# SandraLouise/SVJedi-graph

Measured on AMD Instinct MI355X. Metric: GAF alignments classified/sec (classify + count all-reduce + genotype, text resident in HBM), higher is better.
Workload: dtype u8/int64 (classify), f64 (likelihood)

## Files before the change

### include/svjg.h

```cpp
#ifndef SVJG_H
#define SVJG_H

#include <stdint.h>

#ifdef __cplusplus
extern "C" {
#endif

#define SVJG_ABI_VERSION 1

#define SVJG_E_NO_DEVICE   (-1)
#define SVJG_E_HIP         (-2)
#define SVJG_E_ARG         (-3)
#define SVJG_E_NOMEM       (-4)
#define SVJG_E_RCCL        (-5)
#define SVJG_E_IO          (-6)
#define SVJG_E_INPUT       (-10)
#define SVJG_E_OVERFLOW    (-12)

#define SVJG_EXC_NONE            0
#define SVJG_EXC_VALUE_ERROR     1
#define SVJG_EXC_INDEX_ERROR     2
#define SVJG_EXC_KEY_ERROR       3
#define SVJG_EXC_ZERO_DIVISION   4
#define SVJG_EXC_ASK_HOST        5
#define SVJG_EXC_TYPE_ERROR      6

typedef struct svjg_ctx svjg_ctx;

#define SVJG_LEN_UNKNOWN 0xFFFFFFFFu
#define SVJG_NODE_HAZARD 1u

typedef struct {
    uint64_t key;
    uint32_t aux;
    uint32_t row;
} svjg_node;

typedef struct {
    uint32_t right;
    uint32_t meta;
    uint32_t h0;
    uint32_t h1;
} svjg_edge;

typedef struct {
    const svjg_node *nodes;        uint64_t n_nodes;
    const svjg_edge *edges;        uint64_t n_edges;
    const uint32_t  *hits;         uint64_t n_hits;
    const char      *chrom_names;  const uint32_t *chrom_off;  const uint32_t *chrom_node_lo;  uint32_t n_chrom;
    uint32_t         n_slots;
    uint32_t         d_over;
    uint32_t         flags;
} svjg_graph;

#define SVJG_GRAPH_ALL_SLOW 1u
#define SVJG_GRAPH_DOVER_LIST 16u

typedef struct {
    uint64_t line_start;
    uint32_t slot;
    uint16_t n_ref;
    uint16_t n_alt;
} svjg_hitrec;

typedef struct {
    uint64_t n_lines;
    uint64_t n_deferred;
    uint64_t n_hitrecs;
    uint64_t non_ascii;
} svjg_stats;

int  svjg_abi_version(void);
int  svjg_device_count(void);
int  svjg_init(int device, svjg_ctx **out);
void svjg_destroy(svjg_ctx *ctx);
const char *svjg_last_error(const svjg_ctx *ctx);

int svjg_load_graph(svjg_ctx *ctx, const svjg_graph *g);
void svjg_release_host_tables(void);

int svjg_gaf_upload(svjg_ctx *ctx, const char *gaf, uint64_t n_bytes);
int svjg_gaf_upload_file(svjg_ctx *ctx, const char *path, uint64_t offset, uint64_t n_bytes);
int svjg_gaf_upload_part(svjg_ctx *ctx, const char *gaf, uint64_t n_bytes, uint64_t offset, uint64_t capacity_bytes, int last);
int svjg_classify_resident(svjg_ctx *ctx, uint64_t base_offset, int want_hits);
int svjg_classify(svjg_ctx *ctx, const char *gaf, uint64_t n_bytes, uint64_t base_offset, int want_hits);
int svjg_classify_file(svjg_ctx *ctx, const char *path, uint64_t offset, uint64_t n_bytes, int want_hits);
int svjg_reset_counts(svjg_ctx *ctx);
int svjg_get_stats(svjg_ctx *ctx, svjg_stats *out);
int svjg_input_error(svjg_ctx *ctx, int *exc_class, uint64_t *line_offset);
int svjg_get_defer_causes(svjg_ctx *ctx, uint64_t *out8);

int svjg_get_counts(svjg_ctx *ctx, uint32_t *out, uint32_t n_slots);
int svjg_set_counts(svjg_ctx *ctx, const uint32_t *in, uint32_t n_slots);
int svjg_alloc_counts(svjg_ctx *ctx, uint32_t n_slots);
int svjg_get_hits(svjg_ctx *ctx, svjg_hitrec *out, uint64_t cap, uint64_t *n);
int svjg_get_host_lines(svjg_ctx *ctx, uint64_t *out, uint64_t cap, uint64_t *n);

int svjg_comm_unique_id(char *out128);
int svjg_comm_init(svjg_ctx *ctx, const char *id128, int n_ranks, int rank);
int svjg_allreduce_counts(svjg_ctx *ctx);
int svjg_comm_init_all(svjg_ctx *const *ctxs, int n);
int svjg_comm_error(char *out, uint64_t cap);
int svjg_comm_set_stream(svjg_ctx *ctx, int second_stream);
int svjg_allreduce_counts_all(svjg_ctx *const *ctxs, int n);

int svjg_genotype(svjg_ctx *ctx, const uint8_t *sv_type, const uint32_t *slot, const uint8_t *ok,
                  uint64_t n_rows, uint32_t min_support, double err,
                  uint8_t *gt, int64_t *pl, uint32_t *raw, uint8_t *genotyped);
int svjg_genotype_boundary(svjg_ctx *ctx, uint8_t *out, uint64_t n_rows);
int svjg_genotype_view(svjg_ctx *ctx, const uint8_t *sv_type, const uint32_t *slot, const uint8_t *ok,
                       uint64_t n_rows, uint32_t min_support, double err,
                       const uint8_t **gt, const int64_t **pl, const uint32_t **raw, const uint8_t **genotyped);

int svjg_set_rows(svjg_ctx *ctx, const uint8_t *sv_type, const uint32_t *slot, const uint8_t *ok, uint64_t n_rows);
int svjg_run_resident(svjg_ctx *ctx, uint64_t base_offset, uint32_t min_support, double err,
                      const uint8_t **gt, const int32_t **pl, const uint32_t **raw, const uint8_t **flags, const uint8_t **boundary);
int svjg_run_begin(svjg_ctx *ctx, uint64_t base_offset, uint32_t min_support, double err);
int svjg_run_end(svjg_ctx *ctx, const uint8_t **gt, const int32_t **pl, const uint32_t **raw, const uint8_t **flags, const uint8_t **boundary);

int svjg_write_informative_json(const char *path, const char *gaf, uint64_t n_bytes, const svjg_hitrec *recs,
                                uint64_t n_recs, const char *const *sv_ids, uint32_t n_slots, int n_threads);

int svjg_count_informative_json(const char *path, char **keys_out, uint64_t *keys_len, uint64_t **counts_out, uint64_t *n_keys);
void svjg_host_free(void *p);

#define SVJG_E_UNSUPPORTED (-11)
typedef struct svjg_hostgraph svjg_hostgraph;
int  svjg_graph_load(const char *edges_json_path, const char *gfa_path, svjg_hostgraph **out);
const svjg_graph *svjg_graph_view(const svjg_hostgraph *g);
int  svjg_graph_info(const svjg_hostgraph *g, const char **sv_ids_blob, uint64_t *sv_ids_len, uint32_t *n_hazard);
void svjg_graph_free(svjg_hostgraph *g);

typedef struct svjg_vcf svjg_vcf;
int  svjg_vcf_load(const char *vcf_path, const char *keys_blob, uint64_t blob_len, const uint32_t *slots, uint32_t n_keys,
                   int slot_is_presence, svjg_vcf **out);
int  svjg_vcf_arrays(const svjg_vcf *v, const uint8_t **sv_type, const uint32_t **slot, const uint8_t **ok, uint64_t *n_rows);
int  svjg_vcf_write(const svjg_vcf *v, const char *out_path, const uint8_t *gt, const int64_t *pl, const uint32_t *raw,
                    const uint8_t *genotyped, uint64_t *n_genotyped);
void svjg_vcf_free(svjg_vcf *v);

int svjg_last_kernel_ms(svjg_ctx *ctx, float *classify_main_ms, float *classify_slow_ms, float *genotype_ms);
int svjg_sync(svjg_ctx *ctx);
int svjg_copy_rate(svjg_ctx *ctx, uint64_t n_bytes, double *copy_gb_per_s, double *read_gb_per_s);

#ifdef __cplusplus
}
#endif
#endif
```

### svjedi-graph_amd/csrc/svjg_capi.hip

```cpp
#include "svjg_kernels.h"
#include "svjg_host_tables.h"
#include "svjg_pass.h"
#include <rccl/rccl.h>
#include <errno.h>
#include <math.h>
#include <stdio.h>
#include <stdlib.h>
#include <string.h>
#include <fcntl.h>
#include <unistd.h>
#include <string>
#include <thread>
#include <vector>

using namespace svjg;
typedef struct svjg_ctx svjg_ctx;

static thread_local std::string g_init_error;

#include <memory>
#include <mutex>
namespace {
struct TablesCache {
    std::mutex mu;
    uint64_t key[6] = {0, 0, 0, 0, 0, 0};
    std::shared_ptr<const KernelTables> kt;
} g_tables;

uint64_t fold64(const void *p, size_t n, uint64_t h) {
    const uint8_t *b = (const uint8_t *)p;
    for (size_t i = 0; i + 8 <= n; i += 8) { uint64_t w; memcpy(&w, b + i, 8); h = (h ^ w) * 0x9E3779B97F4A7C15ull; h ^= h >> 29; }
    if (n & 7) { uint64_t w = 0; memcpy(&w, b + (n & ~(size_t)7), n & 7); h = (h ^ w ^ ((uint64_t)(n & 7) << 56)) * 0x9E3779B97F4A7C15ull; h ^= h >> 29; }
    return h;
}

uint64_t graph_digest(const svjg_graph &g, uint64_t seed) {
    uint64_t h = seed;
    h = fold64(g.nodes, (size_t)(g.n_nodes + 1) * sizeof(svjg_node), h);
    h = fold64(g.edges, (size_t)g.n_edges * sizeof(svjg_edge), h ^ g.n_edges);
    h = fold64(g.hits, (size_t)g.n_hits * sizeof(uint32_t), h ^ g.n_hits);
    h = fold64(g.chrom_off, (size_t)(g.n_chrom + 1) * sizeof(uint32_t), h ^ g.n_chrom);
    h = fold64(g.chrom_node_lo, (size_t)(g.n_chrom + 1) * sizeof(uint32_t), h);
    h = fold64(g.chrom_names, (size_t)g.chrom_off[g.n_chrom], h);
    const uint64_t tail[3] = {g.d_over, g.flags, g.n_slots};
    return fold64(tail, sizeof tail, h);
}

std::shared_ptr<const KernelTables> kernel_tables_for(const svjg_graph &g) {
    const uint64_t key[6] = {g.n_nodes, g.n_edges, g.n_hits, g.n_chrom, graph_digest(g, 1), graph_digest(g, 0xD6E8FEB86659FD93ull)};
    std::lock_guard<std::mutex> lk(g_tables.mu);
    if (!g_tables.kt || memcmp(key, g_tables.key, sizeof key) != 0) {
        g_tables.kt = std::make_shared<const KernelTables>(build_kernel_tables(g));
        memcpy(g_tables.key, key, sizeof key);
    }
    return g_tables.kt;
}
}

extern "C" void svjg_release_host_tables(void) {
    std::lock_guard<std::mutex> lk(g_tables.mu);
    g_tables.kt.reset();
    memset(g_tables.key, 0, sizeof g_tables.key);
}

constexpr int STAGE_THREADS = 4;
constexpr uint64_t STAGE_PIECE = 8ull << 20;

struct svjg_ctx {
    int device = 0;
    int n_cu = 256;
    int occ_main = 0;
    hipStream_t stream = nullptr, copy_stream = nullptr;
    hipEvent_t ev[6] = {};
    std::string err;
    bool have_graph = false, have_counts = false;
    svjg_node *d_nodes = nullptr;  svjg_edge *d_edges = nullptr;  uint32_t *d_hits = nullptr;
    uint8_t *d_cnames = nullptr;   uint32_t *d_coff = nullptr, *d_clo = nullptr, *d_chash = nullptr, *d_names = nullptr, *d_links = nullptr, *d_nok = nullptr;  uint16_t *d_disp = nullptr;  uint32_t *d_ihits = nullptr, *d_pfx = nullptr;
    GraphView gv{};
    uint32_t names_len = 0, gflags = 0, n_slots = 0;
    unsigned long long *d_counts = nullptr, *d_snap = nullptr;
    uint8_t *d_gaf = nullptr;  uint64_t gaf_cap = 0, gaf_bytes = 0;  bool have_gaf = false;
    char *h_stage[STAGE_THREADS * 2] = {};
    hipStream_t stage_stream[STAGE_THREADS] = {};
    hipEvent_t stage_ev[STAGE_THREADS * 2] = {};
    uint64_t *d_deferred = nullptr;  uint64_t deferred_cap = 0;
    svjg_hitrec *d_recs = nullptr;   uint64_t rec_cap = 0;
    uint64_t *d_host = nullptr;      uint64_t host_cap = 0;
    DevStatus *d_st = nullptr;
    unsigned long long *d_dbg = nullptr;
    uint32_t *d_long = nullptr;
    DevStatus *h_stp = nullptr;
    DevStatus &hs() { return *h_stp; }
    uint64_t total_deferred = 0;
    dd *d_logfact = nullptr;  uint32_t logfact_n = 0;  dd *d_bsum = nullptr;
    unsigned int *d_maxn = nullptr;
    void *d_rows = nullptr;  uint64_t rows_cap = 0;
    void *h_rows = nullptr;  uint64_t h_rows_cap = 0;
    uint64_t geno_rows = 0;
    struct RunSlot {
        void *d = nullptr;  uint64_t d_cap = 0;  void *h = nullptr;  uint64_t h_cap = 0;  void *h_dev = nullptr;
        unsigned long long *counts = nullptr;  uint64_t counts_cap = 0;
        hipEvent_t ev[6] = {};  hipEvent_t computed = nullptr, copied = nullptr;
        uint64_t base_offset = 0;  uint32_t min_support = 0;  double err = 0;  bool had_text = false, slow_end_own = false;
    } run[2];
    int run_head = 0, run_tail = 0, run_inflight = 0;
    int counts_in_slot = -1;
    void *d_run_in = nullptr;  uint64_t d_run_in_cap = 0;  uint64_t run_rows = 0;  bool have_rows = false;
    float ms_main = 0, ms_slow = 0, ms_geno = 0;
    ncclComm_t comm = nullptr;
    bool allreduce_second = false;
    uint64_t part_total = 0, part_need = 0, part_next = 0;
};

#define HIPCHK(ctx, call)                                                                         \
    do {                                                                                          \
        hipError_t e_ = (call);                                                                   \
        if (e_ != hipSuccess) {                                                                   \
            (ctx)->err = std::string(#call) + ": " + hipGetErrorString(e_);                       \
            return SVJG_E_HIP;                                                                    \
        }                                                                                         \
    } while (0)

extern "C" int svjg_abi_version(void) { return SVJG_ABI_VERSION; }

extern "C" int svjg_device_count(void) {
    int n = 0;
    if (hipGetDeviceCount(&n) != hipSuccess) return 0;
    return n;
}

extern "C" const char *svjg_last_error(const svjg_ctx *ctx) { return ctx ? ctx->err.c_str() : g_init_error.c_str(); }

extern "C" int svjg_init(int device, svjg_ctx **out) {
    if (!out) return SVJG_E_ARG;
    *out = nullptr;
    int n = 0;
    hipError_t e = hipGetDeviceCount(&n);
    if (e != hipSuccess || n <= 0) {
        g_init_error = "no HIP device visible (libsvjg_hip has no CPU fallback)";
        return SVJG_E_NO_DEVICE;
    }
    if (device < 0 || device >= n) { g_init_error = "device index out of range"; return SVJG_E_ARG; }
    svjg_ctx *c = new svjg_ctx();
    c->device = device;
    if (hipSetDevice(device) != hipSuccess || hipStreamCreate(&c->stream) != hipSuccess) {
        g_init_error = "hipSetDevice / hipStreamCreate failed";
        delete c;
        return SVJG_E_HIP;
    }
    hipDeviceProp_t prop;
    if (hipGetDeviceProperties(&prop, device) == hipSuccess) c->n_cu = prop.multiProcessorCount;
    for (auto &ev : c->ev) hipEventCreate(&ev);
    if (hipMalloc(&c->d_dbg, 32 * 8) != hipSuccess || hipMalloc(&c->d_st, sizeof(DevStatus)) != hipSuccess || hipMalloc(&c->d_maxn, sizeof(unsigned int)) != hipSuccess ||
        hipHostMalloc((void **)&c->h_stp, 2 * sizeof(DevStatus), hipHostMallocDefault) != hipSuccess) {
        g_init_error = "hipMalloc failed";
        delete c;
        return SVJG_E_NOMEM;
    }
    memset(c->h_stp, 0, 2 * sizeof(DevStatus));
    c->h_stp[1].err = ~0ull;
    hipFuncSetAttribute((const void *)k_classify_main, hipFuncAttributeMaxDynamicSharedMemorySize, 160 * 1024);
    *out = c;
    return 0;
}

static void free_graph(svjg_ctx *c) {
    hipFree(c->d_nodes); hipFree(c->d_edges); hipFree(c->d_hits); hipFree(c->d_cnames); hipFree(c->d_coff);
    hipFree(c->d_clo); hipFree(c->d_chash); hipFree(c->d_counts); hipFree(c->d_snap); hipFree(c->d_names); hipFree(c->d_links); hipFree(c->d_disp); hipFree(c->d_ihits); hipFree(c->d_nok); hipFree(c->d_pfx);
    c->d_pfx = nullptr; c->d_nok = nullptr; c->d_names = nullptr; c->d_links = nullptr; c->d_disp = nullptr; c->d_ihits = nullptr;
    c->d_nodes = nullptr; c->d_edges = nullptr; c->d_hits = nullptr; c->d_cnames = nullptr; c->d_coff = nullptr;
    c->d_clo = nullptr; c->d_chash = nullptr; c->d_counts = nullptr; c->d_snap = nullptr;
    c->have_graph = false; c->have_counts = false;
}

extern "C" void svjg_destroy(svjg_ctx *c) {
    if (!c) return;
    hipSetDevice(c->device);
    if (c->stream) hipStreamSynchronize(c->stream);
    if (c->copy_stream) hipStreamSynchronize(c->copy_stream);
    if (c->comm) ncclCommDestroy(c->comm);
    free_graph(c);
    hipFree(c->d_long);
    hipFree(c->d_gaf); hipFree(c->d_deferred); hipFree(c->d_recs); hipFree(c->d_host); hipFree(c->d_st); hipFree(c->d_logfact);
    hipFree(c->d_bsum); hipFree(c->d_maxn); hipFree(c->d_rows); hipFree(c->d_run_in);
    for (auto &r : c->run) {
        hipFree(r.d); hipFree(r.counts);
        if (r.h) hipHostFree(r.h);
        for (auto &e : r.ev) if (e) hipEventDestroy(e);
        if (r.computed) hipEventDestroy(r.computed);
        if (r.copied) hipEventDestroy(r.copied);
    }
    if (c->h_rows) hipHostFree(c->h_rows);
    if (c->h_stp) hipHostFree(c->h_stp);
    for (auto &b : c->h_stage) if (b) hipHostFree(b);
    for (auto &ev : c->stage_ev) if (ev) hipEventDestroy(ev);
    for (auto &st : c->stage_stream) if (st) hipStreamDestroy(st);
    for (auto &ev : c->ev) if (ev) hipEventDestroy(ev);
    if (c->copy_stream) hipStreamDestroy(c->copy_stream);
    if (c->stream) hipStreamDestroy(c->stream);
    delete c;
}

template <class T>
static int upload(svjg_ctx *c, T **dst, const T *src, uint64_t n, uint64_t extra = 0) {
    HIPCHK(c, hipMalloc((void **)dst, (n + extra + 1) * sizeof(T)));
    if (n) HIPCHK(c, hipMemcpyAsync(*dst, src, n * sizeof(T), hipMemcpyHostToDevice, c->stream));
    return 0;
}

#ifndef SVJG_SMALL_CHUNK
#define SVJG_SMALL_CHUNK 65536
#endif
#ifndef SVJG_FIRST_SHARE
#define SVJG_FIRST_SHARE 0.85
#endif
constexpr uint64_t SMALL_CHUNK = SVJG_SMALL_CHUNK;
constexpr double FIRST_CHUNK_SHARE = SVJG_FIRST_SHARE;

static int reset_status(svjg_ctx *c, bool all) {
    if (all) {
        c->hs() = c->h_stp[1]; c->total_deferred = 0;
        HIPCHK(c, hipMemcpyAsync(c->d_st, &c->h_stp[1], sizeof(DevStatus), hipMemcpyHostToDevice, c->stream));
        return 0;
    }
    c->hs().n_deferred = 0; c->hs().overflow = 0; c->hs().next_chunk = 0;
    HIPCHK(c, hipMemcpyAsync(c->d_st, &c->hs(), sizeof(DevStatus), hipMemcpyHostToDevice, c->stream));
    return 0;
}

extern "C" int svjg_load_graph(svjg_ctx *c, const svjg_graph *g) {
    if (!c || !g || !g->nodes || !g->chrom_off || !g->chrom_node_lo) return SVJG_E_ARG;
    if (g->n_nodes >= 0x7FFFFFFFull || g->n_edges >= 0x7FFFFFFFull || g->n_chrom >= 65535) { c->err = "graph too large"; return SVJG_E_ARG; }
    if (g->d_over >= 0x80000000u) { c->err = "d_over too large"; return SVJG_E_ARG; }
    HIPCHK(c, hipSetDevice(c->device));
    free_graph(c);
    int rc;
    struct Undo { svjg_ctx *c; bool armed = true; ~Undo() { if (armed) { hipStreamSynchronize(c->stream); free_graph(c); } } } undo{c};
    if ((rc = upload(c, &c->d_nodes, g->nodes, g->n_nodes + 1))) return rc;
    if ((rc = upload(c, &c->d_edges, g->edges, g->n_edges))) return rc;
    if ((rc = upload(c, &c->d_hits, g->hits, g->n_hits))) return rc;
    c->names_len = g->chrom_off[g->n_chrom];
    if ((rc = upload(c, &c->d_cnames, (const uint8_t *)g->chrom_names, c->names_len, 8))) return rc;
    if ((rc = upload(c, &c->d_coff, g->chrom_off, g->n_chrom + 1))) return rc;
    if ((rc = upload(c, &c->d_clo, g->chrom_node_lo, g->n_chrom + 1))) return rc;
    std::vector<uint32_t> hash = build_chrom_hash(*g);
    if ((rc = upload(c, &c->d_chash, hash.data(), hash.size()))) return rc;
    const std::shared_ptr<const KernelTables> ktp = kernel_tables_for(*g);
    const KernelTables &kt = *ktp;
    if ((rc = upload(c, &c->d_names, kt.names.data(), kt.names.size()))) return rc;
    if ((rc = upload(c, &c->d_links, kt.links.data(), kt.links.size()))) return rc;
    if ((rc = upload(c, &c->d_disp, kt.disp.data(), kt.disp.size()))) return rc;
    if ((rc = upload(c, &c->d_ihits, kt.ihits.data(), kt.ihits.size()))) return rc;
    if ((rc = upload(c, &c->d_nok, kt.node_of_kid.data(), kt.node_of_kid.size()))) return rc;
    if (!kt.name_pfx.empty() && (rc = upload(c, &c->d_pfx, kt.name_pfx.data(), kt.name_pfx.size()))) return rc;
    HIPCHK(c, hipStreamSynchronize(c->stream));
    c->gv.nodes = c->d_nodes; c->gv.n_nodes = (uint32_t)g->n_nodes; c->gv.edges = c->d_edges; c->gv.hits = c->d_hits;
    c->gv.chrom_names = c->d_cnames; c->gv.chrom_off = c->d_coff; c->gv.chrom_lo = c->d_clo; c->gv.chrom_hash = c->d_chash;
    c->gv.n_chrom = g->n_chrom; c->gv.hash_mask = (uint32_t)hash.size() - 1; c->gv.d_over = g->d_over;
    c->gv.dover_list = (g->flags & SVJG_GRAPH_DOVER_LIST) ? 1u : 0u;
    c->gv.name_pfx = c->d_pfx;
    c->gv.node_of_kid = c->d_nok; c->gv.name_tab = c->d_names; c->gv.name_ihits = c->d_ihits; c->gv.name_disp = c->d_disp; c->gv.name_slots = kt.name_slots; c->gv.name_buckets = kt.name_buckets;
    c->gv.name_complete = (kt.names_left_out == 0 && kt.names_skipped == 0) ? 1u : 0u;
    c->gv.link_tab = c->d_links; c->gv.link_mask = kt.link_mask; c->gv.link_seed = kt.link_seed;
    c->gflags = g->flags;
    if (g->flags & SVJG_GRAPH_DOVER_LIST) c->gflags |= SVJG_GRAPH_ALL_SLOW;
    if (kt.links_left_out) c->gflags |= SVJG_GRAPH_ALL_SLOW;
    c->n_slots = g->n_slots;
    HIPCHK(c, hipMalloc((void **)&c->d_counts, ((uint64_t)g->n_slots + GUARD_WORDS) * 8));
    HIPCHK(c, hipMalloc((void **)&c->d_snap, ((uint64_t)g->n_slots + GUARD_WORDS) * 8));
    c->have_graph = true; c->have_counts = true;
    undo.armed = false;
    return svjg_reset_counts(c);
}

extern "C" int svjg_alloc_counts(svjg_ctx *c, uint32_t n_slots) {
    if (!c) return SVJG_E_ARG;
    HIPCHK(c, hipSetDevice(c->device));
    free_graph(c);
    c->n_slots = n_slots;
    HIPCHK(c, hipMalloc((void **)&c->d_counts, ((uint64_t)n_slots + GUARD_WORDS) * 8));
    HIPCHK(c, hipMalloc((void **)&c->d_snap, ((uint64_t)n_slots + GUARD_WORDS) * 8));
    c->have_counts = true;
    return svjg_reset_counts(c);
}

extern "C" int svjg_reset_counts(svjg_ctx *c) {
    if (!c || !c->have_counts) return SVJG_E_ARG;
    c->counts_in_slot = -1;
    HIPCHK(c, hipSetDevice(c->device));
    HIPCHK(c, hipMemsetAsync(c->d_counts, 0, ((uint64_t)c->n_slots + GUARD_WORDS) * 8, c->stream));
    return reset_status(c, true);
}

static int gaf_reserve(svjg_ctx *c, uint64_t n, uint64_t *need_out) {
    const uint64_t need = ((n + 15) & ~15ull) + TEXT + 64;
    if (need > c->gaf_cap) {
        HIPCHK(c, hipStreamSynchronize(c->stream));
        hipFree(c->d_gaf); c->d_gaf = nullptr; c->gaf_cap = 0;
        HIPCHK(c, hipMalloc((void **)&c->d_gaf, need));
        c->gaf_cap = need;
    }
    *need_out = need;
    return 0;
}

static int staged_upload(svjg_ctx *c, int fd, uint64_t offset, uint64_t n, uint64_t dst_off = 0) {
    for (int i = 0; i < STAGE_THREADS * 2; ++i) {
        if (!c->h_stage[i]) HIPCHK(c, hipHostMalloc((void **)&c->h_stage[i], STAGE_PIECE, hipHostMallocDefault));
        if (!c->stage_ev[i]) HIPCHK(c, hipEventCreateWithFlags(&c->stage_ev[i], hipEventDisableTiming));
    }
    for (int t = 0; t < STAGE_THREADS; ++t)
        if (!c->stage_stream[t]) HIPCHK(c, hipStreamCreateWithFlags(&c->stage_stream[t], hipStreamNonBlocking));
    const uint64_t n_pieces = (n + STAGE_PIECE - 1) / STAGE_PIECE;
    std::string errs[STAGE_THREADS];
    int rcs[STAGE_THREADS] = {};
    auto feeder = [&](int t) {
        auto fail = [&](int rc, const std::string &m) { rcs[t] = rc; errs[t] = m; };
        if (hipSetDevice(c->device) != hipSuccess) return fail(SVJG_E_HIP, "hipSetDevice in an ingest thread");
        bool used[2] = {false, false};
        uint64_t k = 0;
        for (uint64_t p = (uint64_t)t; p < n_pieces && !rcs[t]; p += STAGE_THREADS, ++k) {
            const int b = t * 2 + (int)(k & 1);
            const uint64_t a = p * STAGE_PIECE, len = n - a < STAGE_PIECE ? n - a : STAGE_PIECE;
            if (used[k & 1] && hipEventSynchronize(c->stage_ev[b]) != hipSuccess) return fail(SVJG_E_HIP, "hipEventSynchronize (ingest)");
            for (uint64_t got = 0; got < len;) {
                const ssize_t r = pread(fd, c->h_stage[b] + got, len - got, (off_t)(offset + a + got));
                if (r <= 0) return fail(SVJG_E_IO, r == 0 ? "the GAF file is shorter than announced" : std::string("pread: ") + strerror(errno));
                got += (uint64_t)r;
            }
            if (hipMemcpyAsync(c->d_gaf + dst_off + a, c->h_stage[b], len, hipMemcpyHostToDevice, c->stage_stream[t]) != hipSuccess ||
                hipEventRecord(c->stage_ev[b], c->stage_stream[t]) != hipSuccess) return fail(SVJG_E_HIP, "hipMemcpyAsync (ingest)");
            used[k & 1] = true;
        }
        if (hipStreamSynchronize(c->stage_stream[t]) != hipSuccess) fail(SVJG_E_HIP, "hipStreamSynchronize (ingest)");
    };
    std::vector<std::thread> th;
    for (int t = 1; t < STAGE_THREADS; ++t) th.emplace_back(feeder, t);
    feeder(0);
    for (auto &x : th) x.join();
    for (int t = 0; t < STAGE_THREADS; ++t)
        if (rcs[t]) { c->err = errs[t]; return rcs[t]; }
    return 0;
}

static uint32_t lane_blocks_per_cu(svjg_ctx *c) {
    static int per_cu = 0;
    if (!per_cu) {
        int n = 0;
        if (hipOccupancyMaxActiveBlocksPerMultiprocessor(&n, k_classify_slow, (int)SLOW_TPB, 0) != hipSuccess || n < 1) n = 4;
        per_cu = n;
    }
    (void)c;
    return (uint32_t)per_cu;
}

static int gaf_finish(svjg_ctx *c, uint64_t n, uint64_t need) {
    HIPCHK(c, hipMemsetAsync(c->d_gaf + n, 0, need - n, c->stream));
    HIPCHK(c, hipStreamSynchronize(c->stream));
    c->gaf_bytes = n;
    c->have_gaf = true;
    return 0;
}

extern "C" int svjg_gaf_upload(svjg_ctx *c, const char *gaf, uint64_t n) {
    if (!c || (n && !gaf)) return SVJG_E_ARG;
    if (c->run_inflight) { c->err = "svjg_gaf_upload with a pass in flight (svjg_run_end first: a repeat of that pass would read the new text)"; return SVJG_E_ARG; }
    HIPCHK(c, hipSetDevice(c->device));
    uint64_t need;
    int rc = gaf_reserve(c, n, &need);
    if (rc) return rc;
    c->have_gaf = false;
    if (n) HIPCHK(c, hipMemcpyAsync(c->d_gaf, gaf, n, hipMemcpyHostToDevice, c->stream));
    return gaf_finish(c, n, need);
}

extern "C" int svjg_gaf_upload_part(svjg_ctx *c, const char *gaf, uint64_t n, uint64_t offset, uint64_t capacity, int last) {
    if (!c || (n && !gaf) || n > capacity || offset > capacity - n) return SVJG_E_ARG;
    if (c->run_inflight) { c->err = "svjg_gaf_upload_part with a pass in flight (svjg_run_end first)"; return SVJG_E_ARG; }
    HIPCHK(c, hipSetDevice(c->device));
    if (offset == 0) {
        int rc = gaf_reserve(c, capacity, &c->part_need);
        if (rc) return rc;
        c->have_gaf = false; c->part_total = capacity; c->part_next = 0;
    }
    if (capacity != c->part_total || offset != c->part_next || c->have_gaf) { c->err = "svjg_gaf_upload_part: pieces go in ascending order, the first at offset 0"; return SVJG_E_ARG; }
    if (n) HIPCHK(c, hipMemcpyAsync(c->d_gaf + offset, gaf, n, hipMemcpyHostToDevice, c->stream));
    HIPCHK(c, hipStreamSynchronize(c->stream));
    c->part_next = offset + n;
    if (last) return gaf_finish(c, c->part_next, c->part_need);
    return 0;
}

extern "C" int svjg_gaf_upload_file(svjg_ctx *c, const char *path, uint64_t offset, uint64_t n) {
    if (!c || !path) return SVJG_E_ARG;
    if (c->run_inflight) { c->err = "svjg_gaf_upload_file with a pass in flight (svjg_run_end first)"; return SVJG_E_ARG; }
    HIPCHK(c, hipSetDevice(c->device));
    uint64_t need;
    int rc = gaf_reserve(c, n, &need);
    if (rc) return rc;
    c->have_gaf = false;
    if (n) {
        const int fd = open(path, O_RDONLY | O_CLOEXEC);
        if (fd < 0) { c->err = std::string("open ") + path + ": " + strerror(errno); return SVJG_E_IO; }
        rc = staged_upload(c, fd, offset, n);
        close(fd);
        if (rc) return rc;
    }
    return gaf_finish(c, n, need);
}

static int ensure(svjg_ctx *c, void **p, uint64_t *cap, uint64_t want, size_t elem, bool keep) {
    if (want <= *cap) return 0;
    const uint64_t asked = want;
    if (keep && *cap && want < *cap + *cap / 2) want = *cap + *cap / 2;
    void *q = nullptr;
    if (want != asked && hipMalloc(&q, want * elem) != hipSuccess) { (void)hipGetLastError(); q = nullptr; want = asked; }
    if (!q) HIPCHK(c, hipMalloc(&q, want * elem));
    if (keep && *p && *cap) HIPCHK(c, hipMemcpyAsync(q, *p, *cap * elem, hipMemcpyDeviceToDevice, c->stream));
    HIPCHK(c, hipStreamSynchronize(c->stream));
    hipFree(*p);
    *p = q; *cap = want;
    return 0;
}

static int fetch_slot_counts(svjg_ctx *c) {
    if (c->counts_in_slot < 0) return 0;
    const int k = c->counts_in_slot;
    c->counts_in_slot = -1;
    HIPCHK(c, hipSetDevice(c->device));
    if (c->run[k].copied) HIPCHK(c, hipStreamWaitEvent(c->stream, c->run[k].copied, 0));
    HIPCHK(c, hipMemcpyAsync(c->d_counts, c->run[k].counts, ((uint64_t)c->n_slots + GUARD_WORDS) * 8, hipMemcpyDeviceToDevice, c->stream));
    return 0;
}

static uint64_t deferred_want(const svjg_ctx *c, uint64_t n) { return (c->gflags & SVJG_GRAPH_ALL_SLOW) ? n / 24 + 64 : (n / 4096 + 65536); }

static void main_launch_setup(svjg_ctx *c, uint64_t begin, uint64_t end, uint64_t base_offset, int want_hits, ClassifyArgs &a, uint32_t &grid, size_t &lds) {
    const uint64_t n = end - begin;
    const bool all_slow = (c->gflags & SVJG_GRAPH_ALL_SLOW) != 0;
    a.gaf = c->d_gaf; a.begin = begin; a.n_bytes = end; a.base_offset = base_offset; a.g = c->gv;
    a.all_slow = all_slow; a.want_hits = want_hits != 0;
#ifdef SVJG_ABLATE
    { const char *dg = getenv("SVJG_DIAG"); a.diag = dg ? (uint32_t)atoi(dg) : 0u; }
#endif
    a.counts = c->d_counts; a.deferred = c->d_deferred; a.deferred_cap = c->deferred_cap;
    a.recs = c->d_recs; a.rec_cap = c->rec_cap; a.host_lines = c->d_host; a.host_cap = c->host_cap; a.st = c->d_st; a.dbg = c->d_dbg;
    lds = LDS_MAIN;
    if (c->occ_main < 1) {
        int occ = 0;
        if (hipOccupancyMaxActiveBlocksPerMultiprocessor(&occ, k_classify_main, (int)WG, lds) != hipSuccess || occ < 1) occ = 1;
        const int by_lds = (int)((160u * 1024u) / ((lds + LDS_GRANULE - 1) / LDS_GRANULE * LDS_GRANULE));
        if (by_lds >= 1 && occ > by_lds) occ = by_lds;
        c->occ_main = occ;
        hipFree(c->d_long); c->d_long = nullptr;
#ifdef SVJG_ABLATE
        { const char *oc = getenv("SVJG_OCC"); fprintf(stderr, "[svjg diag] occupancy API: %d workgroups of %u threads per CU (LDS %zu)\n", occ, WG, lds); if (oc && atoi(oc) > 0) c->occ_main = atoi(oc); }
#endif
    }
    const uint64_t full = (uint64_t)c->n_cu * (uint64_t)c->occ_main;
    if (!c->d_long && hipMalloc((void **)&c->d_long, full * LONG_WORDS * sizeof(uint32_t)) != hipSuccess) c->d_long = nullptr;
    a.long_pre = c->d_long;
    const uint64_t share = (n + full - 1) / full;
    uint64_t region = (share + 15) & ~15ull;
    a.small = 0;
    if (share >= 8 * SMALL_CHUNK) { region = ((uint64_t)(share * FIRST_CHUNK_SHARE) + 15) & ~15ull; a.small = SMALL_CHUNK; }
    if (region < TEXT) region = TEXT;
    a.region = region;
    const uint64_t want_grid = (n + region - 1) / region;
    grid = (uint32_t)(want_grid < full ? want_grid : full);
}

static int classify_range(svjg_ctx *c, uint64_t begin, uint64_t end, uint64_t base_offset, int want_hits) {
    HIPCHK(c, hipSetDevice(c->device));
    { const int rc0 = fetch_slot_counts(c); if (rc0) return rc0; }
    if (end <= begin) return 0;
    const uint64_t n = end - begin;
    uint64_t def_want = deferred_want(c, n);
    uint64_t rec_want = want_hits ? c->hs().n_recs + n / 40 + 65536 : 0;
    uint64_t host_want = c->hs().n_host + 4096;
    int rc;
    for (int attempt = 0; attempt < 3; ++attempt) {
        if ((rc = ensure(c, (void **)&c->d_deferred, &c->deferred_cap, def_want, sizeof(uint64_t), false))) return rc;
        if ((rc = ensure(c, (void **)&c->d_host, &c->host_cap, host_want, sizeof(uint64_t), true))) return rc;
        if (want_hits && (rc = ensure(c, (void **)&c->d_recs, &c->rec_cap, rec_want, sizeof(svjg_hitrec), true))) return rc;
        HIPCHK(c, hipMemcpyAsync(c->d_snap, c->d_counts, ((uint64_t)c->n_slots + GUARD_WORDS) * 8, hipMemcpyDeviceToDevice, c->stream));
        DevStatus before = c->hs();
        if ((rc = reset_status(c, false))) return rc;
        ClassifyArgs a{};
        uint32_t grid = 0;
        size_t lds = 0;
        main_launch_setup(c, begin, end, base_offset, want_hits, a, grid, lds);
        if (!a.long_pre) { c->err = "no memory for the workers' scratch words"; return SVJG_E_NOMEM; }
#ifdef SVJG_TIMING
        if (a.diag & 16u) HIPCHK(c, hipMemsetAsync(c->d_dbg, 0, 32 * 8, c->stream));
#endif
        HIPCHK(c, hipEventRecord(c->ev[0], c->stream));
        hipLaunchKernelGGL(k_classify_main, dim3(grid), dim3(WG), lds, c->stream, a);
        HIPCHK(c, hipGetLastError());
        HIPCHK(c, hipEventRecord(c->ev[1], c->stream));
        HIPCHK(c, hipMemcpyAsync(&c->hs(), c->d_st, sizeof(DevStatus), hipMemcpyDeviceToHost, c->stream));
        HIPCHK(c, hipStreamSynchronize(c->stream));
        const uint64_t n_def = c->hs().n_deferred;
#ifdef SVJG_TIMING
        if (a.diag & 16u) {
            unsigned long long d[16];
            HIPCHK(c, hipMemcpy(d, c->d_dbg, sizeof d, hipMemcpyDeviceToHost));
// ... 283 lines not shown
    std::lock_guard<std::mutex> lk(g_comm_err_mu);
    const size_t n = g_comm_err.size() < cap - 1 ? g_comm_err.size() : (size_t)cap - 1;
    memcpy(out, g_comm_err.data(), n); out[n] = 0;
    return 0;
}

extern "C" int svjg_comm_init_all(svjg_ctx *const *ctxs, int n) {
    if (!ctxs || n < 1 || n > 64) return SVJG_E_ARG;
    for (int i = 0; i < n; ++i) if (!ctxs[i]) return SVJG_E_ARG;
    if (n == 1) return 0;
    int devs[64];
    ncclComm_t comms[64];
    for (int i = 0; i < n; ++i) {
        devs[i] = ctxs[i]->device;
        for (int j = 0; j < i; ++j) if (devs[j] == devs[i]) { comm_err_set("svjg_comm_init_all: one context per device"); return SVJG_E_ARG; }
    }
    ncclResult_t r = ncclCommInitAll(comms, n, devs);
    if (r != ncclSuccess) { comm_err_set(std::string("ncclCommInitAll: ") + ncclGetErrorString(r)); return SVJG_E_RCCL; }
    for (int i = 0; i < n; ++i) {
        if (ctxs[i]->comm) ncclCommDestroy(ctxs[i]->comm);
        ctxs[i]->comm = comms[i];
    }
    return 0;
}

extern "C" int svjg_allreduce_counts_all(svjg_ctx *const *ctxs, int n) {
    if (!ctxs || n < 1 || n > 64) return SVJG_E_ARG;
    for (int i = 0; i < n; ++i) {
        if (!ctxs[i] || !ctxs[i]->have_counts || ctxs[i]->n_slots != ctxs[0]->n_slots) return SVJG_E_ARG;
        if (n > 1 && !ctxs[i]->comm) { ctxs[0]->err = "svjg_comm_init_all has not been called"; return SVJG_E_ARG; }
    }
    int rc;
    for (int i = 0; i < n; ++i) if ((rc = fetch_slot_counts(ctxs[i])) || (rc = launch_guard(ctxs[i]))) { if (i) ctxs[0]->err = ctxs[i]->err; return rc; }
    if (n > 1) {
        ncclResult_t r = ncclGroupStart();
        for (int i = 0; i < n && r == ncclSuccess; ++i) {
            svjg_ctx *c = ctxs[i];
            if (hipSetDevice(c->device) != hipSuccess) { ctxs[0]->err = "hipSetDevice"; ncclGroupEnd(); return SVJG_E_HIP; }
            r = ncclAllReduce(c->d_counts, c->d_counts, (size_t)c->n_slots + GUARD_WORDS, ncclUint64, ncclSum, c->comm, c->stream);
        }
        const ncclResult_t r2 = ncclGroupEnd();
        if (r == ncclSuccess) r = r2;
        if (r != ncclSuccess) { ctxs[0]->err = std::string("ncclAllReduce (group): ") + ncclGetErrorString(r); return SVJG_E_RCCL; }
    }
    for (int i = 0; i < n; ++i) if ((rc = check_guard(ctxs[i]))) { if (i) ctxs[0]->err = ctxs[i]->err; return rc; }
    return 0;
}


static int build_logfact(svjg_ctx *c, uint32_t upto) {
    if (upto > LOGFACT_CAP) upto = LOGFACT_CAP;
    const uint32_t want = (upto + LF_BLOCK - 1) / LF_BLOCK * LF_BLOCK;
    hipFree(c->d_logfact); hipFree(c->d_bsum); c->d_logfact = nullptr; c->d_bsum = nullptr; c->logfact_n = 0;
    HIPCHK(c, hipMalloc((void **)&c->d_logfact, (uint64_t)want * sizeof(dd)));
    HIPCHK(c, hipMalloc((void **)&c->d_bsum, (uint64_t)(want / LF_BLOCK) * sizeof(dd)));
    hipLaunchKernelGGL(k_logfact_local, dim3(want / LF_BLOCK), dim3(LF_BLOCK), 0, c->stream, c->d_logfact, c->d_bsum, want);
    hipLaunchKernelGGL(k_logfact_bsum, dim3(1), dim3(64), 0, c->stream, c->d_bsum, want / LF_BLOCK);
    hipLaunchKernelGGL(k_logfact_add, dim3(want / LF_BLOCK), dim3(LF_BLOCK), 0, c->stream, c->d_logfact, c->d_bsum, want);
    HIPCHK(c, hipGetLastError());
    c->logfact_n = want;
    return 0;
}

static int genotype_rows(svjg_ctx *c, const uint8_t *sv_type, const uint32_t *slot, const uint8_t *ok, uint64_t n_rows,
                         uint32_t min_support, double err) {
    HIPCHK(c, hipSetDevice(c->device));
    { const int rc0 = fetch_slot_counts(c); if (rc0) return rc0; }
    const uint64_t out_bytes = n_rows * 35, maxn_off = (out_bytes + 7) & ~7ull, in_off = maxn_off + 8, in_bytes = n_rows * 6;
    const uint64_t total = in_off + in_bytes + 64;
    int rc = ensure(c, &c->d_rows, &c->rows_cap, total, 1, false);
    if (rc) return rc;
    if (total > c->h_rows_cap) {
        if (c->h_rows) hipHostFree(c->h_rows);
        c->h_rows = nullptr; c->h_rows_cap = 0;
        HIPCHK(c, hipHostMalloc(&c->h_rows, total, hipHostMallocDefault));
        c->h_rows_cap = total;
    }
    uint8_t *base = (uint8_t *)c->d_rows, *hb = (uint8_t *)c->h_rows;
    int64_t *d_pl = (int64_t *)base;
    uint32_t *d_raw = (uint32_t *)(base + n_rows * 24);
    uint8_t *d_gt = base + n_rows * 32, *d_done = base + n_rows * 33;
    unsigned int *d_maxn = (unsigned int *)(base + maxn_off);
    uint32_t *d_slot = (uint32_t *)(base + in_off);
    uint8_t *d_type = base + in_off + n_rows * 4, *d_ok = base + in_off + n_rows * 5;
    memcpy(hb + in_off, slot, n_rows * 4); memcpy(hb + in_off + n_rows * 4, sv_type, n_rows); memcpy(hb + in_off + n_rows * 5, ok, n_rows);
    HIPCHK(c, hipMemcpyAsync(base + in_off, hb + in_off, in_bytes, hipMemcpyHostToDevice, c->stream));
    GenoArgs a{};
    a.counts = c->d_counts; a.sv_type = d_type; a.slot = d_slot; a.ok = d_ok; a.n_rows = n_rows; a.min_support = min_support;
    a.l_ok = log10(1.0 - err); a.l_err = log10(err); a.l_half = log10(1.0 / 2.0);
    a.gt = d_gt; a.pl = d_pl; a.raw = d_raw; a.genotyped = d_done; a.boundary = base + n_rows * 34; a.max_n = d_maxn; a.n_slots = c->n_slots;
    c->geno_rows = n_rows;
    const uint32_t grid = (uint32_t)((n_rows + TPB - 1) / TPB);
    HIPCHK(c, hipEventRecord(c->ev[4], c->stream));
    uint32_t grow_to = 65536;
    for (int attempt = 0; attempt < 2; ++attempt) {
        if (c->logfact_n == 0 && (rc = build_logfact(c, grow_to))) return rc;
        a.logfact = c->d_logfact; a.logfact_n = c->logfact_n;
        HIPCHK(c, hipMemsetAsync(d_maxn, 0, 8, c->stream));
        hipLaunchKernelGGL(k_genotype, dim3(grid), dim3(TPB), 0, c->stream, a);
        HIPCHK(c, hipGetLastError());
        if (attempt == 0) HIPCHK(c, hipEventRecord(c->ev[5], c->stream));
        HIPCHK(c, hipMemcpyAsync(hb, base, maxn_off + 8, hipMemcpyDeviceToHost, c->stream));
        HIPCHK(c, hipStreamSynchronize(c->stream));
        if (*(const unsigned int *)(hb + maxn_off + 4)) { c->err = "slot out of range"; return SVJG_E_ARG; }
        const unsigned int max_n = *(const unsigned int *)(hb + maxn_off);
        if (max_n == 0) break;
        if (attempt == 1) { c->err = "log10(i!) table could not be sized"; return SVJG_E_HIP; }
        grow_to = max_n < LOGFACT_CAP - 1024 ? max_n + 1 + 1024 : LOGFACT_CAP;
        c->logfact_n = 0;
    }
    HIPCHK(c, hipEventElapsedTime(&c->ms_geno, c->ev[4], c->ev[5]));
    return 0;
}

extern "C" int svjg_genotype(svjg_ctx *c, const uint8_t *sv_type, const uint32_t *slot, const uint8_t *ok, uint64_t n_rows,
                             uint32_t min_support, double err, uint8_t *gt, int64_t *pl, uint32_t *raw, uint8_t *genotyped) {
    if (!c || !c->have_counts) return SVJG_E_ARG;
    if (n_rows == 0) return 0;
    if (!sv_type || !slot || !ok || !gt || !pl || !raw || !genotyped) return SVJG_E_ARG;
    const int rc = genotype_rows(c, sv_type, slot, ok, n_rows, min_support, err);
    if (rc) return rc;
    const uint8_t *hb = (const uint8_t *)c->h_rows;
    memcpy(pl, hb, n_rows * 24); memcpy(raw, hb + n_rows * 24, n_rows * 8);
    memcpy(gt, hb + n_rows * 32, n_rows); memcpy(genotyped, hb + n_rows * 33, n_rows);
    return 0;
}

extern "C" int svjg_genotype_view(svjg_ctx *c, const uint8_t *sv_type, const uint32_t *slot, const uint8_t *ok, uint64_t n_rows,
                                  uint32_t min_support, double err, const uint8_t **gt, const int64_t **pl, const uint32_t **raw,
                                  const uint8_t **genotyped) {
    if (!c || !c->have_counts || !gt || !pl || !raw || !genotyped) return SVJG_E_ARG;
    *gt = nullptr; *pl = nullptr; *raw = nullptr; *genotyped = nullptr;
    if (n_rows == 0) return 0;
    if (!sv_type || !slot || !ok) return SVJG_E_ARG;
    const int rc = genotype_rows(c, sv_type, slot, ok, n_rows, min_support, err);
    if (rc) return rc;
    const uint8_t *hb = (const uint8_t *)c->h_rows;
    *pl = (const int64_t *)hb; *raw = (const uint32_t *)(hb + n_rows * 24);
    *gt = hb + n_rows * 32; *genotyped = hb + n_rows * 33;
    return 0;
}

struct RunLayout { uint64_t pl32, raw, gt, flags, boundary, h_tail, out_bytes;  uint64_t maxn, status, guard, tail_bytes, pl64, total; };
static RunLayout run_layout(uint64_t n) {
    RunLayout L; uint64_t o = 0;
    L.pl32 = o; o += n * 12; L.raw = o; o += n * 8; L.gt = o; o += n; L.flags = o; o += n; L.boundary = o; o += n; o = (o + 63) & ~63ull; L.h_tail = o;
    uint64_t d = 0;
    L.maxn = d; d += 8; L.status = d; d += (sizeof(DevStatus) + 7) & ~7ull; L.guard = d; d += GUARD_WORDS * 8; L.tail_bytes = d;
    L.out_bytes = L.h_tail + L.tail_bytes;
    d = (d + 63) & ~63ull; L.pl64 = d; d += n * 24; L.total = d + 64;
    return L;
}

extern "C" int svjg_set_rows(svjg_ctx *c, const uint8_t *sv_type, const uint32_t *slot, const uint8_t *ok, uint64_t n_rows) {
    if (!c || (n_rows && (!sv_type || !slot || !ok))) return SVJG_E_ARG;
    if (c->run_inflight) { c->err = "svjg_set_rows with a pass in flight"; return SVJG_E_ARG; }
    if (!c->have_counts) { c->err = "svjg_set_rows needs the count vector (svjg_load_graph / svjg_alloc_counts first)"; return SVJG_E_ARG; }
    { const int rc0 = fetch_slot_counts(c); if (rc0) return rc0; }
    HIPCHK(c, hipSetDevice(c->device));
    const RunLayout L = run_layout(n_rows);
    int rc;
    if ((rc = ensure(c, &c->d_run_in, &c->d_run_in_cap, n_rows * 6 + 64, 1, false))) return rc;
    for (int k = 0; k < 2; ++k) {
        svjg_ctx::RunSlot &r = c->run[k];
        if ((rc = ensure(c, &r.d, &r.d_cap, L.total, 1, false))) return rc;
        if (L.out_bytes > r.h_cap) {
            if (r.h) hipHostFree(r.h);
            r.h = nullptr; r.h_cap = 0;
            HIPCHK(c, hipHostMalloc(&r.h, L.out_bytes, hipHostMallocMapped));
            r.h_cap = L.out_bytes;
            HIPCHK(c, hipHostGetDevicePointer(&r.h_dev, r.h, 0));
        }
        if ((rc = ensure(c, (void **)&r.counts, &r.counts_cap, (uint64_t)c->n_slots + GUARD_WORDS, sizeof(unsigned long long), false))) return rc;
        for (auto &e : r.ev) if (!e) HIPCHK(c, hipEventCreate(&e));
        if (!r.computed) HIPCHK(c, hipEventCreate(&r.computed));
        if (!r.copied) HIPCHK(c, hipEventCreateWithFlags(&r.copied, hipEventDisableTiming));
    }
    if (!c->copy_stream) {
        int least = 0, greatest = 0;
        if (hipDeviceGetStreamPriorityRange(&least, &greatest) != hipSuccess) least = 0;
        HIPCHK(c, hipStreamCreateWithPriority(&c->copy_stream, hipStreamNonBlocking, least));
    }
    uint8_t *in = (uint8_t *)c->d_run_in;
    if (n_rows) {
        HIPCHK(c, hipMemcpyAsync(in, slot, n_rows * 4, hipMemcpyHostToDevice, c->stream));
        HIPCHK(c, hipMemcpyAsync(in + n_rows * 4, sv_type, n_rows, hipMemcpyHostToDevice, c->stream));
        HIPCHK(c, hipMemcpyAsync(in + n_rows * 5, ok, n_rows, hipMemcpyHostToDevice, c->stream));
    }
    HIPCHK(c, hipStreamSynchronize(c->stream));
    c->run_rows = n_rows; c->have_rows = true;
    return 0;
}

static GenoArgs run_geno_args(svjg_ctx *c, const svjg_ctx::RunSlot &r, const RunLayout &L, uint32_t min_support, double err, const unsigned long long *counts) {
    uint8_t *base = (uint8_t *)r.d, *hostb = (uint8_t *)r.h_dev;
    const uint8_t *in = (const uint8_t *)c->d_run_in;
    GenoArgs a{};
    a.counts = counts; a.slot = (const uint32_t *)in; a.sv_type = in + c->run_rows * 4; a.ok = in + c->run_rows * 5; a.n_rows = c->run_rows;
    a.min_support = min_support;
    a.l_ok = log10(1.0 - err); a.l_err = log10(err); a.l_half = log10(1.0 / 2.0);
    a.gt = hostb + L.gt; a.pl = (int64_t *)(base + L.pl64); a.raw = (uint32_t *)(hostb + L.raw); a.genotyped = hostb + L.flags;
    a.pl32 = (int32_t *)(hostb + L.pl32); a.boundary = hostb + L.boundary; a.max_n = (unsigned int *)(base + L.maxn); a.n_slots = c->n_slots;
    a.logfact = c->d_logfact; a.logfact_n = c->logfact_n;
    return a;
}

extern "C" int svjg_run_begin(svjg_ctx *c, uint64_t base_offset, uint32_t min_support, double err) {
    if (!c) return SVJG_E_ARG;
    if (!c->have_graph || !c->have_gaf) { c->err = "svjg_run_begin needs a graph and an uploaded GAF"; return SVJG_E_ARG; }
    if (!c->have_rows) { c->err = "svjg_set_rows has not been called"; return SVJG_E_ARG; }
    if (c->run_inflight >= 2) { c->err = "two passes are in flight: svjg_run_end first"; return SVJG_E_ARG; }
    HIPCHK(c, hipSetDevice(c->device));
    const uint64_t n = c->gaf_bytes, n_rows = c->run_rows;
    const RunLayout L = run_layout(n_rows);
    svjg_ctx::RunSlot &r = c->run[c->run_head];
    int rc;
    if ((rc = ensure(c, (void **)&c->d_deferred, &c->deferred_cap, deferred_want(c, n), sizeof(uint64_t), false))) return rc;
    if ((rc = ensure(c, (void **)&c->d_host, &c->host_cap, 4096, sizeof(uint64_t), false))) return rc;
    if (c->logfact_n == 0 && (rc = build_logfact(c, 65536))) return rc;
    r.base_offset = base_offset; r.min_support = min_support; r.err = err;
    uint8_t *base = (uint8_t *)r.d;
    DevStatus *d_st = (DevStatus *)(base + L.status);
    if (r.counts_cap < (uint64_t)c->n_slots + GUARD_WORDS) { c->err = "svjg_set_rows must follow svjg_load_graph"; return SVJG_E_ARG; }
    GenoArgs ga = run_geno_args(c, r, L, min_support, err, r.counts);
    {
        const uint64_t words = (uint64_t)c->n_slots + GUARD_WORDS;
        uint32_t rg = (uint32_t)((words + TPB - 1) / TPB);
        if (rg > 1024) rg = 1024;
        hipLaunchKernelGGL(k_step_reset, dim3(rg), dim3(TPB), 0, c->stream, r.counts, words, d_st, ga.max_n);
    }
    const uint64_t max_blocks = (uint64_t)c->n_cu * 4, wave_limit = 16 * max_blocks;
    if (n) {
        ClassifyArgs a{};
        uint32_t grid = 0;
        size_t lds = 0;
        main_launch_setup(c, 0, n, base_offset, 0, a, grid, lds);
        if (!a.long_pre) { c->err = "no memory for the workers' scratch words"; return SVJG_E_NOMEM; }
        a.st = d_st; a.counts = r.counts;
        HIPCHK(c, hipEventRecord(r.ev[0], c->stream));
        hipLaunchKernelGGL(k_classify_main, dim3(grid), dim3(WG), lds, c->stream, a);
        HIPCHK(c, hipEventRecord(r.ev[1], c->stream));
        hipLaunchKernelGGL(k_classify_slow_wave, dim3((uint32_t)c->n_cu), dim3(SLOW_TPB), 0, c->stream, a, SLOW_ASK_DEVICE, 0ull, wave_limit);
        const uint64_t lane_blocks = (uint64_t)c->n_cu * lane_blocks_per_cu(c);
        hipLaunchKernelGGL(k_classify_slow, dim3((uint32_t)lane_blocks), dim3(SLOW_TPB), 0, c->stream, a, SLOW_ASK_DEVICE, wave_limit, ~0ull - 1);
        HIPCHK(c, hipGetLastError());
    }
    static const bool env_second = [] { const char *e = getenv("SVJG_ALLREDUCE_STREAM"); return e && !strcmp(e, "second"); }();
    const bool allreduce_second = env_second || c->allreduce_second;
    auto reduce_on = [&](hipStream_t st) -> int {
        int rc2 = launch_guard(c, r.counts, st, d_st);
        if (rc2) return rc2;
        ncclResult_t nr = ncclAllReduce(r.counts, r.counts, (size_t)c->n_slots + GUARD_WORDS, ncclUint64, ncclSum, c->comm, st);
        if (nr != ncclSuccess) { c->err = std::string("ncclAllReduce: ") + ncclGetErrorString(nr); return SVJG_E_RCCL; }
        HIPCHK(c, hipMemcpyAsync(base + L.guard, r.counts + c->n_slots, GUARD_WORDS * 8, hipMemcpyDeviceToDevice, st));
        return 0;
    };
    r.slow_end_own = false;
    if (c->comm && !allreduce_second) {
        if (r.had_text) { HIPCHK(c, hipEventRecord(r.ev[2], c->stream)); r.slow_end_own = true; }
        if ((rc = reduce_on(c->stream))) return rc;
    }
    HIPCHK(c, hipEventRecord(r.computed, c->stream));
    HIPCHK(c, hipStreamWaitEvent(c->copy_stream, r.computed, 0));
    if (c->comm && allreduce_second && (rc = reduce_on(c->copy_stream))) return rc;
    if (n_rows) {
        HIPCHK(c, hipEventRecord(r.ev[4], c->copy_stream));
        uint32_t gb = 64, gg = (uint32_t)c->n_cu;
        { const char *e = getenv("SVJG_GENO_BLOCK"); if (e && atoi(e) > 0) gb = (uint32_t)atoi(e); }
        { const char *e = getenv("SVJG_GENO_GRID"); if (e && atoi(e) > 0) gg = (uint32_t)atoi(e); }
        if (gb > TPB) gb = TPB;
        if ((uint64_t)gg * gb > n_rows + gb) gg = (uint32_t)((n_rows + gb - 1) / gb);
        hipLaunchKernelGGL(k_genotype, dim3(gg), dim3(gb), 0, c->copy_stream, ga);
        HIPCHK(c, hipGetLastError());
        HIPCHK(c, hipEventRecord(r.ev[5], c->copy_stream));
    }
    HIPCHK(c, hipMemcpyAsync((uint8_t *)r.h + L.h_tail, r.d, L.tail_bytes, hipMemcpyDeviceToHost, c->copy_stream));
    HIPCHK(c, hipEventRecord(r.copied, c->copy_stream));
    c->counts_in_slot = c->run_head;
    r.had_text = n != 0;
    c->run_head ^= 1; ++c->run_inflight;
    return 0;
}

extern "C" int svjg_run_end(svjg_ctx *c, const uint8_t **gt, const int32_t **pl, const uint32_t **raw, const uint8_t **flags, const uint8_t **boundary) {
    if (!c || !gt || !pl || !raw || !flags || !boundary) return SVJG_E_ARG;
    *gt = nullptr; *pl = nullptr; *raw = nullptr; *flags = nullptr; *boundary = nullptr;
    if (!c->run_inflight) { c->err = "no pass in flight"; return SVJG_E_ARG; }
    HIPCHK(c, hipSetDevice(c->device));
    svjg_ctx::RunSlot &r = c->run[c->run_tail];
    c->run_tail ^= 1; --c->run_inflight;
    const uint64_t n = c->gaf_bytes, n_rows = c->run_rows;
    const RunLayout L = run_layout(n_rows);
    uint8_t *hb = (uint8_t *)r.h;
    int rc;
    HIPCHK(c, hipEventSynchronize(r.copied));
    const uint8_t *tail = hb + L.h_tail;
    c->hs() = *(const DevStatus *)(tail + L.status);
    c->ms_slow = 0;
    if (r.had_text) {
        HIPCHK(c, hipEventElapsedTime(&c->ms_main, r.ev[0], r.ev[1]));
        if (c->hs().n_deferred) HIPCHK(c, hipEventElapsedTime(&c->ms_slow, r.ev[1], r.slow_end_own ? r.ev[2] : r.computed));
    }
    if (n_rows) HIPCHK(c, hipEventElapsedTime(&c->ms_geno, r.ev[4], r.ev[5]));
    bool again = false;
    const unsigned long long *redo_counts = r.counts;
    const unsigned long long *gd = (const unsigned long long *)(tail + L.guard);
    if (pass_repeats(c->comm != nullptr, c->hs().overflow, gd[GUARD_REPEAT])) {
        if ((rc = svjg_reset_counts(c))) return rc;
        rc = classify_range(c, 0, n, r.base_offset, 0);
        if (rc && rc != SVJG_E_INPUT) return rc;
        if (c->comm) { const std::string keep = c->err; const int rc2 = svjg_allreduce_counts(c); if (rc2 && !rc) return rc2; if (rc) c->err = keep; }
        if (rc) return rc;
        again = true; redo_counts = c->d_counts;
    } else {
        c->total_deferred = c->hs().n_deferred;
        if (c->hs().err != ~0ull) return SVJG_E_INPUT;
        if (c->comm && pass_counts_overflowed(gd[GUARD_MAX_REF], gd[GUARD_MAX_ALT])) { c->err = "more than 2^32 informative alignments for one SV"; return SVJG_E_OVERFLOW; }
    }
    if (c->hs().n_host) { c->err = "the text holds lines only the host can decide (non-ASCII digits in a decimal column: svjg_get_host_lines); classify it with svjg_classify"; return SVJG_E_ARG; }
    if (n_rows) {
        for (int attempt = 0;; ++attempt) {
            if (!again) {
                if (*(const unsigned int *)(tail + L.maxn + 4)) { c->err = "slot out of range"; return SVJG_E_ARG; }
                const unsigned int max_n = *(const unsigned int *)(tail + L.maxn);
                if (max_n == 0) break;
                if (attempt == 2) { c->err = "log10(i!) table could not be sized"; return SVJG_E_HIP; }
                HIPCHK(c, hipStreamSynchronize(c->stream));
                HIPCHK(c, hipStreamSynchronize(c->copy_stream));
                if ((rc = build_logfact(c, max_n < LOGFACT_CAP - 1024 ? max_n + 1 + 1024 : LOGFACT_CAP))) return rc;
            }
            again = false;
            GenoArgs ga = run_geno_args(c, r, L, r.min_support, r.err, redo_counts);
            HIPCHK(c, hipMemsetAsync(ga.max_n, 0, 8, c->stream));
            hipLaunchKernelGGL(k_genotype, dim3((uint32_t)((n_rows + TPB - 1) / TPB)), dim3(TPB), 0, c->stream, ga);
            HIPCHK(c, hipGetLastError());
            HIPCHK(c, hipMemcpyAsync(hb + L.h_tail + L.maxn, (uint8_t *)r.d + L.maxn, 8, hipMemcpyDeviceToHost, c->stream));
            HIPCHK(c, hipStreamSynchronize(c->stream));
        }
    }
    *pl = (const int32_t *)(hb + L.pl32); *raw = (const uint32_t *)(hb + L.raw); *gt = hb + L.gt; *flags = hb + L.flags; *boundary = hb + L.boundary;
    return 0;
}

extern "C" int svjg_run_resident(svjg_ctx *c, uint64_t base_offset, uint32_t min_support, double err,
                                 const uint8_t **gt, const int32_t **pl, const uint32_t **raw, const uint8_t **flags, const uint8_t **boundary) {
    if (!c || !gt || !pl || !raw || !flags || !boundary) return SVJG_E_ARG;
    if (c->run_inflight) { c->err = "svjg_run_resident with a pass in flight (svjg_run_end first)"; return SVJG_E_ARG; }
    const int rc = svjg_run_begin(c, base_offset, min_support, err);
    if (rc) return rc;
    return svjg_run_end(c, gt, pl, raw, flags, boundary);
}

extern "C" int svjg_genotype_boundary(svjg_ctx *c, uint8_t *out, uint64_t n_rows) {
    if (!c || (n_rows && !out) || n_rows != c->geno_rows || !c->h_rows) return SVJG_E_ARG;
    memcpy(out, (const uint8_t *)c->h_rows + n_rows * 34, n_rows);
    return 0;
}

extern "C" int svjg_last_kernel_ms(svjg_ctx *c, float *m, float *s, float *g) {
    if (!c) return SVJG_E_ARG;
    if (m) *m = c->ms_main;
    if (s) *s = c->ms_slow;
    if (g) *g = c->ms_geno;
    return 0;
}

extern "C" int svjg_copy_rate(svjg_ctx *c, uint64_t n_bytes, double *copy_gb_per_s, double *read_gb_per_s) {
    if (!c || n_bytes < (1u << 20)) return SVJG_E_ARG;
    HIPCHK(c, hipSetDevice(c->device));
    n_bytes &= ~4095ull;
    uint4 *src = nullptr, *dst = nullptr;
    if (hipMalloc((void **)&src, n_bytes) != hipSuccess || hipMalloc((void **)&dst, n_bytes) != hipSuccess) { hipFree(src); c->err = "svjg_copy_rate: no memory for the two buffers"; return SVJG_E_NOMEM; }
    struct Free { uint4 *a, *b; ~Free() { hipFree(a); hipFree(b); } } fr{src, dst};
    HIPCHK(c, hipMemsetAsync(src, 0x5A, n_bytes, c->stream));
    HIPCHK(c, hipMemsetAsync(dst, 0, n_bytes, c->stream));
    const uint32_t grid = (uint32_t)c->n_cu * 16;
    for (int what = 0; what < 2; ++what) {
        double *out = what ? read_gb_per_s : copy_gb_per_s;
        if (!out) continue;
        float best = 0;
        for (int i = 0; i < 4; ++i) {
            HIPCHK(c, hipEventRecord(c->ev[2], c->stream));
            if (what) hipLaunchKernelGGL(k_read16, dim3(grid), dim3(TPB), 0, c->stream, dst, src, n_bytes / 16);
            else hipLaunchKernelGGL(k_copy16, dim3(grid), dim3(TPB), 0, c->stream, dst, src, n_bytes / 16);
            HIPCHK(c, hipGetLastError());
            HIPCHK(c, hipEventRecord(c->ev[3], c->stream));
            HIPCHK(c, hipStreamSynchronize(c->stream));
            float ms = 0;
            HIPCHK(c, hipEventElapsedTime(&ms, c->ev[2], c->ev[3]));
            if (i && (best == 0 || ms < best)) best = ms;
        }
        *out = best > 0 ? (what ? 1.0 : 2.0) * (double)n_bytes / (best * 1e-3) / 1e9 : 0.0;
    }
    return 0;
}

extern "C" int svjg_sync(svjg_ctx *c) {
    if (!c) return SVJG_E_ARG;
    HIPCHK(c, hipSetDevice(c->device));
    HIPCHK(c, hipStreamSynchronize(c->stream));
    return 0;
}
```

### svjedi-graph_amd/csrc/svjg_kernels.h

```cpp
#pragma once
#include <hip/hip_runtime.h>
#define SVJG_TAB_AS __attribute__((address_space(3)))
#include "svjg_line.h"
#include "svjg_planes.h"
#include "svjg_pass.h"
#include "svjg_geno.h"

namespace svjg {

constexpr uint32_t WG = 64;
constexpr uint32_t TPB = 256;
constexpr uint32_t PIECES = 4;
constexpr uint32_t SPAN = PIECES * 16;
constexpr uint32_t HALF = SPAN * WG;
constexpr uint32_t NHALF = 2;
constexpr uint32_t TEXT = NHALF * HALF;
constexpr uint32_t MAXL = 64;
#ifndef SVJG_CAP_O
#ifdef SVJG_W16
#define SVJG_CAP_O 208
#else
#define SVJG_CAP_O 216
#endif
#endif
constexpr uint32_t CAP_O = SVJG_CAP_O;
constexpr uint32_t KMAX = 64;
#ifdef SVJG_W16
constexpr uint32_t KLONG = KMAX;
#else
constexpr uint32_t KLONG = CAP_O < 255u ? CAP_O : 255u;
#endif
constexpr uint32_t LONG_LOG = 256;
constexpr uint32_t LONG_WORDS = 3 * LONG_LOG;
static_assert(KLONG <= LONG_LOG && KLONG * 4 <= TEXT / 8 + 16, "a long line's per-node words fit their places");
constexpr uint32_t LRW = MAXL;
static_assert(TEXT + 1 < 65535, "text offsets are kept in 16 bits, 0xFFFF = none");

constexpr uint32_t L_TEXT = 0;
#ifdef SVJG_W16
constexpr uint32_t L_TBM = L_TEXT + TEXT + 64;
constexpr uint32_t L_NDBM = L_TBM;
constexpr uint32_t L_RL = L_TBM;
constexpr uint32_t L_OPL = L_TBM + TEXT / 8 + 16;
constexpr uint32_t L_LINE = L_OPL + (CAP_O + 8) * 3;
constexpr uint32_t LDS_MAIN = L_LINE + (MAXL + 8) * 4;
constexpr uint32_t LDS_GRANULE = 1280;
static_assert(LDS_MAIN <= 8 * LDS_GRANULE, "sixteen workers per CU");
static_assert(L_TBM % 16 == 0 && L_OPL % 16 == 0 && L_LINE % 4 == 0, "LDS alignment");
#else
constexpr uint32_t L_NDBM = L_TEXT + TEXT + 64;
constexpr uint32_t L_RL = L_NDBM;
constexpr uint32_t L_TBM = L_NDBM + TEXT / 8 + 16;
constexpr uint32_t L_OPL = L_TBM + TEXT / 8 + 16;
constexpr uint32_t L_LINE = L_OPL + (CAP_O + 8) * 4;
constexpr uint32_t LDS_MAIN = L_LINE + (MAXL + 8) * 4;
constexpr uint32_t LDS_GRANULE = 1280;
static_assert(LRW * 16 <= TEXT / 8 + 16, "the per-line records fit the bitmap they replace");
static_assert(LDS_MAIN <= 9 * LDS_GRANULE, "fourteen workers per CU");
static_assert(L_NDBM % 16 == 0 && L_TBM % 16 == 0 && L_OPL % 16 == 0 && L_LINE % 16 == 0 && L_RL % 16 == 0, "LDS alignment");
#endif

struct DevStatus {
    unsigned long long n_lines;
    unsigned long long n_deferred;
    unsigned long long n_recs;
    unsigned long long err;
    unsigned int non_ascii;
    unsigned int overflow;
    unsigned long long next_chunk;
    unsigned long long n_host;
    unsigned long long cause[8];
};

struct ClassifyArgs {
    const uint8_t *gaf;
    uint64_t begin;
    uint64_t n_bytes;
    uint64_t base_offset;
    GraphView g;
    uint32_t all_slow;
    uint32_t want_hits;
    uint64_t region;
    uint64_t small;
    uint32_t diag;
    unsigned long long *counts;
    uint64_t *deferred;  uint64_t deferred_cap;
    svjg_hitrec *recs;   uint64_t rec_cap;
    uint64_t *host_lines; uint64_t host_cap;
    DevStatus *st;
    unsigned long long *dbg;
    uint32_t *long_pre;
};

__device__ inline uint32_t zero_bytes(uint32_t t) {
    return ~(((t & 0x7F7F7F7Fu) + 0x7F7F7F7Fu) | t | 0x7F7F7F7Fu);
}
__device__ inline uint32_t eq_mask16(uint4 v, uint32_t pat) {
    const uint32_t lo = __builtin_amdgcn_udot4(zero_bytes(v.x ^ pat), 0x08040201u, __builtin_amdgcn_udot4(zero_bytes(v.y ^ pat), 0x80402010u, 0u, false), false);
    const uint32_t hi = __builtin_amdgcn_udot4(zero_bytes(v.z ^ pat), 0x08040201u, __builtin_amdgcn_udot4(zero_bytes(v.w ^ pat), 0x80402010u, 0u, false), false);
    return (lo | (hi << 8)) >> 7;
}

__device__ inline uint32_t wave_incl_scan(uint32_t v) {
    uint32_t x = v;
    asm("s_nop 1\n\tv_add_u32_dpp %0, %0, %0 row_shr:1 row_mask:0xf bank_mask:0xf bound_ctrl:0\n\t"
        "s_nop 1\n\tv_add_u32_dpp %0, %0, %0 row_shr:2 row_mask:0xf bank_mask:0xf bound_ctrl:0\n\t"
        "s_nop 1\n\tv_add_u32_dpp %0, %0, %0 row_shr:4 row_mask:0xf bank_mask:0xf bound_ctrl:0\n\t"
        "s_nop 1\n\tv_add_u32_dpp %0, %0, %0 row_shr:8 row_mask:0xf bank_mask:0xf bound_ctrl:0\n\t"
        "s_nop 1\n\tv_add_u32_dpp %0, %0, %0 row_bcast:15 row_mask:0xa bank_mask:0xf\n\t"
        "s_nop 1\n\tv_add_u32_dpp %0, %0, %0 row_bcast:31 row_mask:0xc bank_mask:0xf"
        : "+v"(x));
    return x;
}
__device__ inline void wave_incl_scan2(uint32_t &x, uint32_t &y) {
#define SVJG_STEP(ctl) "s_nop 0\n\tv_add_u32_dpp %0, %0, %0 " ctl "\n\tv_add_u32_dpp %1, %1, %1 " ctl "\n\t"
    asm("s_nop 0\n\t"
        SVJG_STEP("row_shr:1 row_mask:0xf bank_mask:0xf bound_ctrl:0") SVJG_STEP("row_shr:2 row_mask:0xf bank_mask:0xf bound_ctrl:0")
        SVJG_STEP("row_shr:4 row_mask:0xf bank_mask:0xf bound_ctrl:0") SVJG_STEP("row_shr:8 row_mask:0xf bank_mask:0xf bound_ctrl:0")
        SVJG_STEP("row_bcast:15 row_mask:0xa bank_mask:0xf") SVJG_STEP("row_bcast:31 row_mask:0xc bank_mask:0xf")
        : "+v"(x), "+v"(y));
#undef SVJG_STEP
}
__device__ inline unsigned long long ballot64(bool p) { return __builtin_amdgcn_ballot_w64(p); }
typedef unsigned long long wmask;
#define RARELY(c) __builtin_expect((c) != 0, 0)
__device__ inline wmask m_eq(uint32_t a, uint32_t b) { return __builtin_amdgcn_uicmp(a, b, 32); }
__device__ inline wmask m_ne(uint32_t a, uint32_t b) { return __builtin_amdgcn_uicmp(a, b, 33); }
__device__ inline wmask m_gt(uint32_t a, uint32_t b) { return __builtin_amdgcn_uicmp(a, b, 34); }
__device__ inline wmask m_ge(uint32_t a, uint32_t b) { return __builtin_amdgcn_uicmp(a, b, 35); }
__device__ inline wmask m_lt(uint32_t a, uint32_t b) { return __builtin_amdgcn_uicmp(a, b, 36); }
__device__ inline wmask m_le(uint32_t a, uint32_t b) { return __builtin_amdgcn_uicmp(a, b, 37); }
__device__ inline bool in_mask(wmask m) { return __builtin_amdgcn_inverse_ballot_w64(m); }
__device__ inline uint32_t rdlane(uint32_t v, uint32_t l) { return (uint32_t)__builtin_amdgcn_readlane((int)v, (int)l); }
__device__ inline uint32_t lane_below_or(uint32_t v, uint32_t first) { return (uint32_t)__builtin_amdgcn_update_dpp((int)first, (int)v, 0x138, 0xF, 0xF, false); }
__device__ inline uint32_t lane_below(uint32_t v) { return (uint32_t)__builtin_amdgcn_update_dpp((int)v, (int)v, 0x138, 0xF, 0xF, false); }
__device__ inline uint32_t lane_above(uint32_t v) { return (uint32_t)__builtin_amdgcn_update_dpp((int)v, (int)v, 0x130, 0xF, 0xF, false); }
__device__ inline uint32_t wave_excl_scan(uint32_t v, uint32_t &total) {
    const uint32_t x = wave_incl_scan(v);
    total = (uint32_t)__builtin_amdgcn_readlane((int)x, 63);
    return x - v;
}

enum : uint32_t { ST_NONE = 0, ST_OK = 1, ST_NOHIT = 2, ST_DEFER = 3 };
enum : uint32_t { DC_COLUMNS = 0,
                  DC_IDF = 1,
                  DC_LONG_PATH = 2,
                  DC_NAME = 3,
                  DC_STRIPE = 4,
                  DC_N = 5 };

typedef uint32_t u32_any __attribute__((aligned(1)));
typedef unsigned long long u64_any __attribute__((aligned(1)));
__device__ inline uint64_t name_words_head(const uint8_t *text, uint32_t a0, uint32_t L, bool any_short, uint32_t d[8]) {
    const uint32_t o2 = (uint32_t)min(max((int32_t)L - 8, 0), 16), o1 = o2 >> 1;
    const uint8_t *p = text + a0;
    unsigned long long w0 = *(const u64_any *)p, w1 = *(const u64_any *)(p + o1), w2 = *(const u64_any *)(p + o2);
    if (RARELY(any_short)) {
        const unsigned long long m = L < 8u ? ~(~0ull << (8u * L)) : ~0ull;
        w0 &= m; w1 &= m; w2 &= m;
    }
    d[0] = (uint32_t)w0; d[1] = (uint32_t)(w0 >> 32); d[2] = (uint32_t)w1; d[3] = (uint32_t)(w1 >> 32); d[4] = (uint32_t)w2; d[5] = (uint32_t)(w2 >> 32);
    d[6] = 0u; d[7] = 0u;
    const uint32_t C[6] = {0x9E3779B1u, 0x85EBCA77u, 0xC2B2AE3Du, 0x27D4EB2Fu, 0x165667B1u, 0xD3A2646Du};
    uint64_t h = (uint64_t)L * 0x7FEB352Du;
#pragma unroll
    for (uint32_t i = 0; i < 6; ++i) h += (uint64_t)d[i] * C[i];
    return h;
}
__device__ inline uint64_t name_words_tail(const uint8_t *text, uint32_t a0, uint32_t L, uint32_t d[8]) {
    const unsigned long long w = *(const u64_any *)(text + a0 + (L > 24u ? L - 8u : 0u));
    d[6] = L > 24u ? (uint32_t)w : 0u;
    d[7] = L > 24u ? (uint32_t)(w >> 32) : 0u;
    return (uint64_t)d[6] * 0xFD7046C5u + (uint64_t)d[7] * 0xB55A4F09u;
}
__device__ inline void name_words_far(const uint8_t *text, uint32_t a0, uint32_t L, uint32_t f[4]) {
    const u32_any *w = (const u32_any *)(text + a0 + (L > 40u ? L - 24u : L > 32u ? L - 16u : 0u));
    f[0] = L > 32u ? w[0] : 0u; f[1] = L > 32u ? w[1] : 0u; f[2] = L > 40u ? w[2] : 0u; f[3] = L > 40u ? w[3] : 0u;
}
__device__ inline void name_prefix_lds(const uint8_t *text, uint32_t a0, uint32_t L, uint32_t p[NAME_PFX_WORDS]) {
    const u32_any *w = (const u32_any *)(text + a0);
    const int32_t n = (int32_t)L - (int32_t)(4u * NAME_WORDS);
#pragma unroll
    for (int32_t i = 0; i < (int32_t)NAME_PFX_WORDS; ++i) {
        const int32_t k = n - 4 * i;
        p[i] = k >= 4 ? w[i] : k <= 0 ? 0u : (w[i] & ((1u << (8 * k)) - 1u));
    }
}
__device__ inline uint64_t name_words_tail2(const uint8_t *text, uint32_t a0, uint32_t L) {
    uint32_t f[4];
    name_words_far(text, a0, L, f);
    return (uint64_t)f[0] * 0x94D049BBu + (uint64_t)f[1] * 0xBF58476Du + (uint64_t)f[2] * 0x2545F491u + (uint64_t)f[3] * 0x9FB21C65u;
}

__device__ inline bool name_match(const uint4 r0, const uint4 r1, const uint4 r2, const uint32_t d[8], uint32_t L) {
    uint32_t diff = ((r1.z & NAME_LEN_MASK) ^ (L - 1u)) | (r0.x ^ d[0]) | (r0.y ^ d[1]) | (r0.z ^ d[2]) | (r0.w ^ d[3]) | (r1.x ^ d[4]) | (r1.y ^ d[5]);
    const uint32_t tail = (r2.x ^ d[6]) | (r2.y ^ d[7]);
    diff |= L > 24u ? tail : 0u;
    return diff == 0u;
}

__device__ inline void long_words_sync() {
    __builtin_amdgcn_fence(__ATOMIC_RELEASE, "workgroup");
    __builtin_amdgcn_wave_barrier();
    __builtin_amdgcn_fence(__ATOMIC_ACQUIRE, "workgroup");
}
__device__ inline void wave_sync() {
    __builtin_amdgcn_fence(__ATOMIC_RELEASE, "wavefront");
    __builtin_amdgcn_wave_barrier();
    __builtin_amdgcn_fence(__ATOMIC_ACQUIRE, "wavefront");
}


struct SpanFlags {
    uint32_t high;
    uint32_t idf;
    uint32_t dee_last;
    uint32_t idsum;
};
__device__ inline uint32_t idsum_of(uint32_t pair_lo, uint32_t pair_hi) {
    const uint32_t cnt = (uint32_t)__popc(pair_lo) + (uint32_t)__popc(pair_hi);
    const uint32_t pos = pair_hi ? 63u - (uint32_t)__builtin_clz(pair_hi) : 31u - (uint32_t)__builtin_clz(pair_lo);
    return ((cnt < 3u ? cnt : 3u) << 6) | pos;
}
__device__ inline uint32_t lane_above_or0(uint32_t v) { return (uint32_t)__builtin_amdgcn_update_dpp(0, (int)v, 0x130, 0xF, 0xF, false); }
__device__ inline void classify_span(const ClassifyArgs &a, const uint8_t *text, uint32_t *ndbm, uint32_t *tbm, uint32_t half, uint32_t slot, uint64_t c0, uint32_t V,
                                     unsigned long long &NL, unsigned long long &ORI, SpanFlags &fl) {
    const uint32_t sp = slot * SPAN;
    const uint32_t rot = (slot >> 2) & 3u;
    uint32_t w[16];
#pragma unroll
    for (uint32_t c = 0; c < PIECES; ++c) {
        const uint4 v = *(const uint4 *)(text + sp + ((c + rot) & 3u) * 16);
        w[c * 4 + 0] = v.x; w[c * 4 + 1] = v.y; w[c * 4 + 2] = v.z; w[c * 4 + 3] = v.w;
    }
    span_planes(w);
    const HalfClasses lo = half_classes(w), hi = half_classes(w + 8);
    const uint32_t sel_lo = (0x0B0A0908u - 0x02020202u * rot) & 0x07070707u, sel_hi = sel_lo ^ 0x04040404u;
    auto place = [&](uint32_t l, uint32_t h) -> unsigned long long {
        return (unsigned long long)perm_b32(h, l, sel_lo) | ((unsigned long long)perm_b32(h, l, sel_hi) << 32);
    };
    unsigned long long nl64 = place(lo.nl, hi.nl);
    const unsigned long long tab64 = place(lo.tab, hi.tab), ori64 = place(lo.ori, hi.ori), nd64 = place(lo.nd, hi.nd);
    fl.high |= lo.high | hi.high;
    {
        const unsigned long long dee = place(lo.dee, hi.dee), col = place(lo.colon, hi.colon);
        const uint32_t nxt = lane_above_or0((uint32_t)col);
        const uint32_t s_lo = __builtin_amdgcn_alignbit((uint32_t)(col >> 32), (uint32_t)col, 1), s_hi = __builtin_amdgcn_alignbit(nxt, (uint32_t)(col >> 32), 1);
        const uint32_t pair_lo = (uint32_t)dee & s_lo, pair_hi = (uint32_t)(dee >> 32) & s_hi;
        fl.idf |= pair_lo | pair_hi;
        if (RARELY(m_ne(pair_lo | pair_hi, 0u))) {
            if ((pair_lo | pair_hi) != 0u) fl.idsum |= idsum_of(pair_lo, pair_hi) << (half ? 8 : 0);
        }
        fl.dee_last = (uint32_t)(dee >> 63);
    }
    if ((lo.cr | hi.cr) != 0) {
        unsigned long long cr = place(lo.cr, hi.cr);
        while (cr) {
            const uint32_t b = (uint32_t)__builtin_ctzll(cr); cr &= cr - 1;
            const uint32_t q = sp + b;
            const uint32_t staged = (slot / WG + 1u) * HALF;
            const uint8_t nx = (q + 1 < staged) ? text[q + 1] : ((c0 + q + 1 < a.n_bytes) ? a.gaf[c0 + q + 1] : 0);
            if (nx != '\n') nl64 |= 1ull << b;
        }
    }
    if (sp + SPAN > V) nl64 &= sp >= V ? 0ull : ((1ull << (V - sp)) - 1ull);
#ifndef SVJG_W16
    *(uint2 *)(ndbm + slot * 2) = make_uint2((uint32_t)nd64, (uint32_t)(nd64 >> 32));
#endif
    *(uint2 *)(tbm + slot * 2) = make_uint2((uint32_t)tab64, (uint32_t)(tab64 >> 32));
    NL = nl64; ORI = ori64;
}

__device__ inline uint32_t field_val(const uint8_t *text, uint32_t a, uint32_t n) {
    const u32_any *w = (const u32_any *)(text + a);
    const uint32_t lo0 = w[0] & 0x0F0F0F0Fu;
    const uint32_t hi0 = w[1] & 0x0F0F0F0Fu;
    const uint32_t n8 = n < 8 ? n : 8;
    const unsigned long long x = (((unsigned long long)hi0 << 32) | lo0) << ((8 * (8 - n8)) & 63u);
    const uint32_t lo = (uint32_t)x, hi = (uint32_t)(x >> 32);
    const uint32_t pl = (((lo << 3) + (lo << 1)) + (lo >> 8)) & 0x00FF00FFu, ph = (((hi << 3) + (hi << 1)) + (hi >> 8)) & 0x00FF00FFu;
    uint32_t r = __umul24(__umul24(pl & 0xFFu, 100u) + (pl >> 16), 10000u) + __umul24(ph & 0xFFu, 100u) + (ph >> 16);
    if (n == 9) r = r * 10u + ((uint32_t)text[a + 8] & 0xFu);
    return r;
}

__device__ inline bool field_is_zero(const uint8_t *text, uint32_t a, uint32_t n) {
    const u32_any *w = (const u32_any *)(text + a);
    const uint32_t lo0 = w[0] & 0x0F0F0F0Fu, hi0 = w[1] & 0x0F0F0F0Fu;
    const uint32_t n8 = n < 8 ? n : 8;
    const unsigned long long x = (((unsigned long long)hi0 << 32) | lo0) << ((8 * (8 - n8)) & 63u);
    return x == 0 && (n < 9 || ((uint32_t)text[a + 8] & 0xFu) == 0);
}

__device__ inline bool bits_clear(const uint32_t *bm, uint32_t a, uint32_t n) {
    const uint32_t *w = bm + (a >> 5);
    const uint32_t sh = a & 31u;
    const unsigned long long lo = (unsigned long long)w[0] | ((unsigned long long)w[1] << 32);
    unsigned long long x = lo >> sh;
    if (sh) x |= (unsigned long long)w[2] << (64u - sh);
    const unsigned long long m = n >= 64u ? ~0ull : ((1ull << n) - 1ull);
    return (x & m) == 0;
}

__device__ inline uint32_t tab_window(const uint32_t *tbm, uint32_t p) {
    const uint32_t *w = tbm + (p >> 5);
    return __builtin_amdgcn_alignbit(w[1], w[0], p & 31u);
}
__device__ inline uint32_t take_tab(uint32_t &win, uint32_t p) {
    const uint32_t t = win ? p + (uint32_t)__builtin_ctz(win) : TEXT;
    win &= win - 1u;
    return t;
}
__device__ inline uint32_t tab_near(const uint32_t *tbm, uint32_t p) {
    const uint32_t win = tab_window(tbm, p);
    return win ? p + (uint32_t)__builtin_ctz(win) : TEXT;
}
__device__ inline uint32_t tab_from(const uint32_t *tbm, uint32_t p, uint32_t lim) {
    for (uint32_t q = p; q < lim; q += 32) {
        const uint32_t win = tab_window(tbm, q);
        if (win) { const uint32_t t = q + (uint32_t)__builtin_ctz(win); return t < lim ? t : TEXT; }
    }
    return TEXT;
}


#ifndef SVJG_P_B2
#define SVJG_P_B2 1
#define SVJG_P_R1 2
#define SVJG_P_LOAD 3
#define SVJG_P_REST 2
#endif
#ifndef SVJG_P_A
#define SVJG_P_A 2
#endif
constexpr int P_A = SVJG_P_A;
constexpr int P_B2 = SVJG_P_B2, P_R1 = SVJG_P_R1, P_LOAD = SVJG_P_LOAD, P_REST = SVJG_P_REST;
#ifdef SVJG_ABLATE
#define DIAG(bit) ((a.diag & (bit)) != 0)
#else
#define DIAG(bit) false
#endif
#ifndef SVJG_MINW
#define SVJG_MINW 4
#endif
__device__ inline unsigned long long low_bits64(uint32_t n) { return n >= 64u ? ~0ull : ((1ull << n) - 1ull); }
__device__ inline uint32_t clamp64(uint32_t hi, uint32_t lo) { return hi > lo ? (hi - lo < 64u ? hi - lo : 64u) : 0u; }

__device__ inline bool long_line_may_repeat(uint32_t *ids, uint32_t K, uint32_t lane) {
    const uint32_t nb = K <= 128u ? 128u : K <= 192u ? 64u : 32u, B = nb * 32u;
    uint32_t *bm = ids + 256u - nb;
    for (uint32_t t = 0; t < 8u; ++t) {
        const uint32_t M = B - t * (B >> 4) - (t ? 2u * t + 1u : 0u);
        const uint32_t inv = 0xFFFFFFFFu / M;
        bm[lane & (nb - 1u)] = 0u;
        if (nb > 64u) bm[64u + lane] = 0u;
        wave_sync();
        uint32_t twice = 0u;
        for (uint32_t m = lane; m < K; m += WG) {
            const uint32_t x = ids[m] & 0x00FFFFFFu;
            uint32_t r = x - __umulhi(x, inv) * M;
            if (r >= M) r -= M;
            const uint32_t was = __hip_atomic_fetch_or(&bm[r >> 5], 1u << (r & 31u), __ATOMIC_RELAXED, __HIP_MEMORY_SCOPE_WAVEFRONT);
            twice |= (was >> (r & 31u)) & 1u;
        }
        if (ballot64(twice != 0u) == 0ull) return false;
        wave_sync();
    }
    return true;
}

__global__ __launch_bounds__(WG, SVJG_MINW) void k_classify_main(ClassifyArgs a) {
    extern __shared__ __attribute__((aligned(16))) uint8_t lds[];
    uint8_t *text = lds + L_TEXT;
    uint32_t *ndbm = (uint32_t *)(lds + L_NDBM);
    uint32_t *tbm = (uint32_t *)(lds + L_TBM);
#ifdef SVJG_W16
    uint16_t *OPLP = (uint16_t *)(lds + L_OPL);
    uint8_t *OPLL = lds + L_OPL + (CAP_O + 8) * 2;
#define OPL_PUT(j, v) do { const uint32_t v_ = (v); OPLP[j] = (uint16_t)v_; OPLL[j] = (uint8_t)((v_ >> 16) + 1u); } while (0)
#define OPL_POS(j) ((uint32_t)OPLP[j])
#else
    uint32_t *OPL = (uint32_t *)(lds + L_OPL);
#define OPL_PUT(j, v) OPL[j] = (v)
#define OPL_POS(j) (OPL[j] & 0xFFFFu)
#endif
    uint32_t *LINE = (uint32_t *)(lds + L_LINE);
    uint4 *RL = (uint4 *)(lds + L_RL);

    const uint32_t lane = threadIdx.x;
    const GraphView g = a.g;

    unsigned long long pos = a.begin + (unsigned long long)blockIdx.x * a.region;
    if (pos >= a.n_bytes) return;
    unsigned long long rend = pos + a.region < a.n_bytes ? pos + a.region : a.n_bytes;

    if (lane < 4) tbm[TEXT / 32 + lane] = 0;
    unsigned long long wave_lines = 0;
#ifdef SVJG_TIMING
    unsigned long long stamp = __builtin_readcyclecounter(), acc[16] = {0, 0, 0, 0, 0, 0, 0, 0, 0, 0, 0, 0, 0, 0, 0, 0};
    auto tick = [&](int ph) { const unsigned long long t = __builtin_readcyclecounter(); acc[ph] += t - stamp; stamp = t; };
#define tick_mem(ph) do { asm volatile("s_waitcnt vmcnt(0) lgkmcnt(0)" ::: "memory"); tick(ph); } while (0)
#define tally(ph, n) do { acc[ph] += (n); } while (0)
#elif defined(SVJG_MARK)
#define tick(ph) asm volatile("; MARK " #ph)
#else
    auto tick = [](int) {};
#endif
#ifndef SVJG_TIMING
#define tick_mem(ph) do { } while (0)
#define tally(ph, n) do { } while (0)
#endif

    constexpr uint32_t NPF = HALF / (WG * 16);
    uint4 pf[NPF];
    uint32_t pf_head = '\n';
    typedef uint32_t u32x4 __attribute__((ext_vector_type(4)));
    auto fetch_half = [&](unsigned long long at) {
        const uint4 *src = (const uint4 *)(a.gaf + at) + lane;
#pragma unroll
        for (uint32_t i = 0; i < NPF; ++i) {
            const u32x4 v = __builtin_nontemporal_load((const u32x4 *)(src + i * WG));
            pf[i] = make_uint4(v.x, v.y, v.z, v.w);
        }
    };
  for (;;) {
    fetch_half(pos & ~15ull);
    { const unsigned long long c0 = pos & ~15ull; pf_head = c0 > a.begin ? a.gaf[c0 - 1] : (uint32_t)'\n'; }

    for (;;) {
        const unsigned long long c0 = pos & ~15ull;
        const uint32_t own_lo = (uint32_t)(pos - c0);
        const uint32_t V = (uint32_t)((a.n_bytes - c0 < (unsigned long long)TEXT) ? (a.n_bytes - c0) : (unsigned long long)TEXT);
        const bool at_eof = c0 + V == a.n_bytes;

        const uint32_t head_byte = pf_head;
        unsigned long long NL[NHALF], ORI[NHALF];
        SpanFlags fl = {0u, 0u, 0u, 0u};
        uint32_t dee_end = 0;
        unsigned long long IDM[NHALF];
#pragma unroll
        for (uint32_t h = 0; h < NHALF; ++h) {
            __builtin_amdgcn_s_setprio(P_A);
#pragma unroll
            for (uint32_t i = 0; i < NPF; ++i) *(uint4 *)(text + h * HALF + (i * WG + lane) * 16) = pf[i];
            if (h + 1 < NHALF) fetch_half(c0 + (h + 1) * HALF);
            wave_sync();
            __builtin_amdgcn_s_setprio(0);
            fl.idf = 0u;
            classify_span(a, text, ndbm, tbm, h, h * WG + lane, c0, V, NL[h], ORI[h], fl);
            IDM[h] = ballot64(fl.idf != 0);
            if (h == 0) dee_end = rdlane(fl.dee_last, WG - 1);
            else if (dee_end != 0 && text[HALF] == ':') {
                IDM[0] |= 1ull << 63;
                if (lane == WG - 1) { const uint32_t c = (fl.idsum >> 6) & 3u; fl.idsum = (fl.idsum & 0xFF00u) | ((c < 3u ? c + 1u : 3u) << 6) | 63u; }
            }
        }
        if (ballot64(fl.high != 0) != 0 && lane == 0) a.st->non_ascii = 1;
        const bool idf = (IDM[0] | IDM[1]) != 0;
        if (idf && lane == 0) {
            LINE[MAXL + 4] = (uint32_t)IDM[0]; LINE[MAXL + 5] = (uint32_t)(IDM[0] >> 32); LINE[MAXL + 6] = (uint32_t)IDM[1]; LINE[MAXL + 7] = (uint32_t)(IDM[1] >> 32);
        }
        tick(0);
        const uint32_t head = (head_byte == '\n') || (head_byte == '\r' && text[0] != '\n');
        uint32_t Vh = V;
        bool eof_h = at_eof;
        uint32_t lim2, n_s, n_own, tot_ori, l_first;
        bool last_stripe, long_line;
        unsigned long long next_pos;
        uint32_t RK[NHALF];
        uint32_t head_own;
        for (uint32_t attempt = 0;; ++attempt) {
            uint32_t s_last = NONE32;
            {
                const unsigned long long b1 = ballot64(NL[1] != 0), b0 = ballot64(NL[0] != 0);
                if (b1 | b0) {
                    const uint32_t hh = b1 ? 1u : 0u;
                    const uint32_t L = 63u - (uint32_t)__builtin_clzll(b1 ? b1 : b0);
                    const uint32_t mlo = (uint32_t)__builtin_amdgcn_readlane((int)(uint32_t)(hh ? NL[1] : NL[0]), (int)L);
                    const uint32_t mhi = (uint32_t)__builtin_amdgcn_readlane((int)(uint32_t)((hh ? NL[1] : NL[0]) >> 32), (int)L);
                    const unsigned long long m = ((unsigned long long)mhi << 32) | mlo;
                    s_last = (hh * WG + L) * SPAN + (63u - (uint32_t)__builtin_clzll(m)) + 1u;
                } else if (head) s_last = 0;
            }
            const uint32_t own_lim = rend - c0 < (unsigned long long)Vh ? (uint32_t)(rend - c0) : Vh;
            lim2 = own_lim;
            last_stripe = false; long_line = false;
            next_pos = c0 + Vh;
            if (eof_h) last_stripe = true;
            else if (s_last == NONE32 || s_last < own_lo) { }
            else if (c0 + s_last >= rend) last_stripe = true;
            else if (s_last > own_lo) { lim2 = s_last; next_pos = c0 + s_last; }
            else long_line = true;
            if (next_pos >= rend) last_stripe = true;

            uint32_t in0 = ((uint32_t)__popcll(NL[0]) + (lane == 0 ? head : 0u)) | ((uint32_t)__popcll(ORI[0]) << 16);
            uint32_t in1 = (uint32_t)__popcll(NL[1]) | ((uint32_t)__popcll(ORI[1]) << 16);
            const uint32_t c0v = in0, c1v = in1;
            wave_incl_scan2(in0, in1);
            const uint32_t tot0 = rdlane(in0, WG - 1), tots = tot0 + rdlane(in1, WG - 1);
            RK[0] = in0 - c0v; RK[1] = tot0 + in1 - c1v;
            n_s = tots & 0xFFFFu; tot_ori = tots >> 16;
            auto starts_before = [&](uint32_t x) -> uint32_t {
                if (x == 0) return 0u;
                const uint32_t q = x - 1u, slot = q >> 6, hh = slot >> 6, L = slot & 63u;
                const uint32_t rk = rdlane(hh ? RK[1] : RK[0], L) & 0xFFFFu;
                const uint32_t mlo = rdlane((uint32_t)(hh ? NL[1] : NL[0]), L), mhi = rdlane((uint32_t)((hh ? NL[1] : NL[0]) >> 32), L);
                const unsigned long long m = (((unsigned long long)mhi << 32) | mlo) & ((1ull << (q & 63u)) - 1ull);
                return rk + (uint32_t)__popcll(m) + (slot == 0 ? head : 0u);
            };
            l_first = starts_before(own_lo);
            n_own = starts_before(lim2) - l_first;
            head_own = head & (uint32_t)(own_lo == 0 && 0 < lim2);
            if (attempt || !(n_s > MAXL || tot_ori > CAP_O)) break;
            uint32_t best[NHALF];
#pragma unroll
            for (uint32_t h = 0; h < NHALF; ++h) {
                const uint32_t sp = (h * WG + lane) * SPAN;
                const uint32_t sb = (RK[h] & 0xFFFFu) + ((h == 0 && lane == 0) ? head : 0u), ob = RK[h] >> 16;
                best[h] = 0;
                for (unsigned long long m = NL[h]; m; m &= m - 1) {
                    const uint32_t b = (uint32_t)__builtin_ctzll(m);
                    const uint32_t ord = sb + (uint32_t)__popcll(NL[h] & ((1ull << b) - 1ull));
                    const uint32_t marks = ob + (uint32_t)__popcll(ORI[h] & ((2ull << b) - 1ull));
                    if (ord + 1u <= MAXL && marks <= CAP_O && sp + b + 1u <= Vh) best[h] = sp + b + 1u;
                }
            }
            uint32_t cut = 0;
            {
                const unsigned long long f1 = ballot64(best[1] != 0), f0 = ballot64(best[0] != 0);
                if (f1) cut = rdlane(best[1], 63u - (uint32_t)__builtin_clzll(f1));
                else if (f0) cut = rdlane(best[0], 63u - (uint32_t)__builtin_clzll(f0));
            }
            if (cut > own_lo && cut > 16u) Vh = cut;
            else if (Vh > HALF) Vh = HALF;
            else break;
            eof_h = false;
#pragma unroll
            for (uint32_t h = 0; h < NHALF; ++h) {
                const unsigned long long keep = low_bits64(clamp64(Vh, (h * WG + lane) * SPAN));
                NL[h] &= keep; ORI[h] &= keep;
            }
        }
        if (RARELY(long_line) && Vh == TEXT && !a.all_slow && tot_ori <= CAP_O && text[TEXT - 1] != 'd') {
            unsigned long long at = c0 + TEXT, E = ~0ull;
            bool clean = true;
// ... 460 lines not shown
                wmask go_m = step_m & m_ge(pre_l, need_l) & m_ge(tot - ((int32_t)fr > (int32_t)lnb ? pre_rx : 0u), need_r);
                uint32_t hold = 0;
                if (RARELY(lsub)) {
                    uint32_t adv = n_pass - 1u;
                    if ((lsub & L_ONE) && !(lsub & L_FINAL)) {
                        const wmask und_m = step_m & m_ge(pre_l, need_l) & ~go_m;
                        if (und_m) adv = (uint32_t)__builtin_ctzll(und_m);
                        if (adv == 0u) {
                            lsub |= L_MEASURE; SET_R(lP);
                            lS += rdlane(gsum, n_pass - 2u); SET_P(lP + n_pass - 1u);
                            continue;
                        }
                        go_m &= low_bits64(adv);
                        hold = (lP << 8) | adv;
                    }
                    if (lsub & L_SWEEP1) go_m &= m_ge(lP + lane, lR);
                    if (!(lsub & L_FINAL)) { lS += rdlane(gsum, adv - 1u); SET_P(lP + adv); }
                }
                const uint32_t want = (idr << 2) | orl | (orr << 1);
                const wmask le24 = m_le(len, 24u), le32 = m_le(len, 32u), le40 = m_le(len, 40u);
                const wmask m0 = le24 & m_eq(r2.x, want), m1 = le32 & m_eq(r2.z, want), m2 = le40 & m_eq(r3.x, want), m3 = m_eq(r3.z, want);
                const wmask inl = m0 | m1 | m2 | m3;
                const uint32_t v = in_mask(m0) ? r2.y : in_mask(m1) ? r2.w : in_mask(m2) ? r3.y : r3.w;
                const wmask found_m = go_m & ~moved_m & inl;
                const wmask ask_m = go_m & (moved_m | ~(inl | m_ne(row_inline, 0u)));
                const bool ask = in_mask(ask_m);
                uint32_t nh = in_mask(found_m) ? 1u : 0u, h0 = v, h1 = 0;
                const uint32_t *hp = nullptr;
                {
                    const wmask many = found_m & m_ge(v, 0x80000000u);
                    if (RARELY(many)) { if (in_mask(many)) { hp = g.name_ihits + (v & 0x7FFFFFFFu) + 1; nh = hp[-1] | 0x80000000u; } }
                }
                if (RARELY(ask_m) && !DIAG(512u)) {
                    const uint64_t hl = h;
                    const uint64_t hr = ((uint64_t)lane_above((uint32_t)(h >> 32)) << 32) | lane_above((uint32_t)h);
                    if (ask) {
                        const uint32_t klo = (idr << 1) | orr, khi = (idl << 1) | orl;
                        uint32_t sa, sb2;
                        link_slots(link_prehash(hl, orl, hr, orr), g.link_seed, g.link_mask, sa, sb2);
                        uint4 ek = *(const uint4 *)(g.link_tab + (size_t)sa * 4);
                        const uint4 ek2 = *(const uint4 *)(g.link_tab + (size_t)sb2 * 4);
                        if (!(ek.x == klo && ek.y == khi)) ek = ek2;
                        if (ek.x == klo && ek.y == khi) {
                            if ((ek.z & 0x80000000u) && ek.w != 0xFFFFFFFFu && ek.z != 0xFFFFFFFFu) { hp = g.hits + (ek.z & 0x7FFFFFFFu); nh = ek.w | 0x80000000u; }
                            else { h0 = ek.z; h1 = ek.w; nh = ek.w == 0xFFFFFFFFu ? 1u : 2u; }
                        }
                    }
                }
                if (RARELY(hold)) {
                    uint32_t hd = hold, lane_c = lane;
                    asm volatile("" : "+s"(hd), "+v"(lane_c));
                    uint32_t *LGw = a.long_pre + (size_t)blockIdx.x * LONG_WORDS + LONG_LOG + 2u * ((hd >> 8) + lane_c);
                    uint32_t w0 = 0xFFFFFFFFu, w1 = 0u;
                    if (nh & 0x80000000u) { w0 = (uint32_t)(hp - (ask ? g.hits : g.name_ihits)); w1 = 0x80000000u | (ask ? 0u : 0x40000000u) | (nh & 0x3FFFFFFFu); }
                    else if (nh) { w0 = h0; w1 = nh == 1u ? 0x7FFFFFFFu : h1; }
                    if (lane_c < (hd & 0xFFu)) {
                        __hip_atomic_store(LGw, w0, __ATOMIC_RELAXED, __HIP_MEMORY_SCOPE_WORKGROUP);
                        __hip_atomic_store(LGw + 1, w1, __ATOMIC_RELAXED, __HIP_MEMORY_SCOPE_WORKGROUP);
                    }
                    nh = 0;
                }
                for (uint32_t fb = 0;;) {
                    unsigned long long rbase = 0;
                    if (RARELY(a.want_hits)) {
                        uint32_t wtot2, ex = wave_excl_scan(nh & 0x7FFFFFFFu, wtot2);
                        if (wtot2) {
                            if (lane == 0) rbase = atomicAdd(&a.st->n_recs, (unsigned long long)wtot2);
                            rbase = __shfl(rbase, 0) + ex;
                        }
                    }
                    auto emit = [&](uint32_t hv, uint32_t jj) {
                        if (!DIAG(8u)) atomicAdd(&((unsigned int *)a.counts)[DIAG(4u) ? (hv & 1023u) : DIAG(64u) ? ((hv & 63u) | ((blockIdx.x & 1023u) << 6)) : hv], 1u);
                        if (a.want_hits) {
                            if (rbase + jj < a.rec_cap) {
                                svjg_hitrec r; r.line_start = a.base_offset + c0 + (LINE[lbase + ln] & 0xFFFFu); r.slot = hv >> 1;
                                r.n_ref = (hv & 1u) ? 0 : 1; r.n_alt = (hv & 1u) ? 1 : 0;
                                a.recs[rbase + jj] = r;
                            } else atomicOr(&a.st->overflow, 2u);
                        }
                    };
                    if (in_mask(m_le(nh - 1u, 1u))) emit(h0, 0);
                    if (RARELY(m_gt(nh, 1u))) {
                        const uint32_t n = nh & 0x7FFFFFFFu;
                        for (uint32_t jj = hp ? 0u : 1u; jj < n; ++jj) emit(hp ? hp[jj] : h1, jj);
                    }
                    if (!RARELY(lsub)) break;
                    if (hold) break;
                    uint32_t ls = lsub, lane_c = lane;
                    asm volatile("" : "+s"(ls), "+v"(lane_c));
                    if (!(ls & L_FINAL)) break;
                    const uint32_t upto = (ls & L_SWEEP1) ? ((ls >> 16) & 0xFFu) : (ls & L_ONE) ? ((ls >> 8) & 0xFFu) : 0u;
                    if (fb >= upto) break;
                    if (fb == 0u) long_words_sync();
                    const uint32_t *LG = a.long_pre + (size_t)blockIdx.x * LONG_WORDS + LONG_LOG + 2u * (fb + lane_c);
                    nh = 0; hp = nullptr;
                    if (fb + lane_c < upto) {
                        const uint32_t w0 = __hip_atomic_load(LG, __ATOMIC_RELAXED, __HIP_MEMORY_SCOPE_WORKGROUP);
                        const uint32_t w1 = __hip_atomic_load(LG + 1, __ATOMIC_RELAXED, __HIP_MEMORY_SCOPE_WORKGROUP);
                        if (w0 != 0xFFFFFFFFu) {
                            if (w1 & 0x80000000u) { hp = ((w1 & 0x40000000u) ? g.name_ihits : g.hits) + w0; nh = (w1 & 0x3FFFFFFFu) | 0x80000000u; }
                            else { h0 = w0; h1 = w1; nh = w1 == 0x7FFFFFFFu ? 1u : 2u; }
                        }
                    }
                    __builtin_amdgcn_s_waitcnt(0x0F70);
                    fb += WG;
                }
                tick(6);
                if (RARELY(lsub) && (lsub & L_FINAL)) { ++i0; lsub = 0; }
            }
#undef lD0
#undef lP
#undef lR
#undef SET_D0
#undef SET_P
#undef SET_R
            wave_sync();
            {
                const uint32_t fin = RL[lane].z >> 24;
                const bool defer = lane < cnt && fin >= ST_DEFER;
                unsigned long long db = ballot64(defer);
                if (RARELY(db)) {
#pragma unroll
                    for (uint32_t cse = 0; cse < DC_STRIPE; ++cse) {
                        const unsigned long long cb = ballot64(defer && fin == ST_DEFER + cse);
                        if (cb && lane == 0) atomicAdd(&a.st->cause[cse], (unsigned long long)__popcll(cb));
                    }
                    unsigned long long dbase = 0;
                    if (lane == 0) dbase = atomicAdd(&a.st->n_deferred, (unsigned long long)__popcll(db));
                    dbase = __shfl(dbase, 0);
                    if (defer) {
                        unsigned long long idx = dbase + __popcll(db & ((1ull << lane) - 1ull));
                        if (idx < a.deferred_cap) a.deferred[idx] = c0 + s; else atomicOr(&a.st->overflow, 1u);
                    }
                }
            }
            wave_sync();
            __builtin_amdgcn_s_setprio(P_R1);
        }
        wave_lines += n_own;
        wave_sync();
        tick(7);
        if (last_stripe) break;
        pos = next_pos;
    }
    if (!a.small) break;
    unsigned long long ci = 0;
    if (lane == 0) ci = atomicAdd(&a.st->next_chunk, 1ull);
    ci = ((unsigned long long)(uint32_t)__builtin_amdgcn_readfirstlane((int)(uint32_t)(ci >> 32)) << 32) | (uint32_t)__builtin_amdgcn_readfirstlane((int)(uint32_t)ci);
    pos = a.begin + (unsigned long long)gridDim.x * a.region + ci * a.small;
    if (pos >= a.n_bytes) break;
    rend = pos + a.small < a.n_bytes ? pos + a.small : a.n_bytes;
  }
    if (lane == 0 && wave_lines) atomicAdd(&a.st->n_lines, wave_lines);
#ifdef SVJG_TIMING
    if ((a.diag & 16u) && lane == 0)
        for (int i = 0; i < 16; ++i) atomicAdd(&a.dbg[i], acc[i]);
#endif
}

typedef uint32_t svjg_u32x4 __attribute__((ext_vector_type(4)));
__global__ __launch_bounds__(TPB) void k_copy16(uint4 *dst, const uint4 *src, uint64_t n16) {
    const uint64_t stride = (uint64_t)gridDim.x * TPB;
    uint64_t i = (uint64_t)blockIdx.x * TPB + threadIdx.x;
    for (; i + 3 * stride < n16; i += 4 * stride) {
        const svjg_u32x4 a = __builtin_nontemporal_load((const svjg_u32x4 *)(src + i)), b = __builtin_nontemporal_load((const svjg_u32x4 *)(src + i + stride));
        const svjg_u32x4 c = __builtin_nontemporal_load((const svjg_u32x4 *)(src + i + 2 * stride)), d = __builtin_nontemporal_load((const svjg_u32x4 *)(src + i + 3 * stride));
        __builtin_nontemporal_store(a, (svjg_u32x4 *)(dst + i)); __builtin_nontemporal_store(b, (svjg_u32x4 *)(dst + i + stride));
        __builtin_nontemporal_store(c, (svjg_u32x4 *)(dst + i + 2 * stride)); __builtin_nontemporal_store(d, (svjg_u32x4 *)(dst + i + 3 * stride));
    }
    for (; i < n16; i += stride) dst[i] = src[i];
}
__global__ __launch_bounds__(TPB) void k_read16(uint4 *sink, const uint4 *src, uint64_t n16) {
    const uint64_t stride = (uint64_t)gridDim.x * TPB;
    uint64_t i = (uint64_t)blockIdx.x * TPB + threadIdx.x;
    uint32_t acc = 0;
    for (; i + 3 * stride < n16; i += 4 * stride) {
        const svjg_u32x4 a = __builtin_nontemporal_load((const svjg_u32x4 *)(src + i)), b = __builtin_nontemporal_load((const svjg_u32x4 *)(src + i + stride));
        const svjg_u32x4 c = __builtin_nontemporal_load((const svjg_u32x4 *)(src + i + 2 * stride)), d = __builtin_nontemporal_load((const svjg_u32x4 *)(src + i + 3 * stride));
        acc ^= a.x ^ a.w ^ b.y ^ b.z ^ c.x ^ c.w ^ d.y ^ d.z;
    }
    for (; i < n16; i += stride) acc ^= src[i].x;
    if (acc == 0x12345677u) sink[0].x = acc;
}

__global__ __launch_bounds__(TPB) void k_step_reset(unsigned long long *counts, uint64_t n_words, DevStatus *st, unsigned int *max_n) {
    for (uint64_t i = (uint64_t)blockIdx.x * TPB + threadIdx.x; i < n_words; i += (uint64_t)gridDim.x * TPB) counts[i] = 0ull;
    if (blockIdx.x == 0 && threadIdx.x == 0) {
        DevStatus z{}; z.err = ~0ull;
        *st = z;
        max_n[0] = 0u; max_n[1] = 0u;
    }
}

__device__ inline void report_line(const ClassifyArgs &a, unsigned long long off, int rc) {
    if (rc == SVJG_EXC_ASK_HOST) {
        const unsigned long long i = atomicAdd(&a.st->n_host, 1ull);
        if (i < a.host_cap) a.host_lines[i] = off; else atomicOr(&a.st->overflow, 4u);
    } else atomicMin(&a.st->err, (off << 3) | (unsigned long long)rc);
}

struct SlowEmit {
    const ClassifyArgs *a;
    uint64_t line_start;
    __device__ void operator()(uint32_t slot, uint32_t allele) {
        atomicAdd(&a->counts[slot], allele ? (1ull << 32) : 1ull);
        if (a->want_hits) {
            unsigned long long idx = atomicAdd(&a->st->n_recs, 1ull);
            if (idx < a->rec_cap) {
                svjg_hitrec r; r.line_start = line_start; r.slot = slot; r.n_ref = allele ? 0 : 1; r.n_alt = allele ? 1 : 0;
                a->recs[idx] = r;
            } else atomicOr(&a->st->overflow, 2u);
        }
    }
};

#ifndef SVJG_SLOW_LANE_LDS
#define SVJG_SLOW_LANE_LDS (16 * 1024)
#endif
constexpr uint32_t SLOW_TPB = 64, SLOW_LDS = 32 * 1024, SLOW_MAXLINE = 16 * 1024;
constexpr uint32_t SLOW_LANE_LDS = SVJG_SLOW_LANE_LDS;
constexpr uint64_t SLOW_ASK_DEVICE = ~0ull;
__device__ inline uint64_t slow_n_def(const ClassifyArgs &a, uint64_t n_def, uint64_t lo, uint64_t hi) {
    if (n_def != SLOW_ASK_DEVICE) return n_def;
    if (a.st->overflow & 1u) return 0;
    const uint64_t n = a.st->n_deferred;
    return (n > lo && n <= hi) ? n : 0;
}
constexpr uint32_t SLOW_LANE_NODES = 12;
__global__ __launch_bounds__(SLOW_TPB) void k_classify_slow(ClassifyArgs a, uint64_t n_def_arg, uint64_t lo, uint64_t hi) {
    const uint64_t n_def = slow_n_def(a, n_def_arg, lo, hi);
    __shared__ __attribute__((aligned(16))) uint8_t stage[SLOW_LANE_LDS];
    __shared__ int64_t c_len[SLOW_LANE_NODES * SLOW_TPB];
    __shared__ uint32_t c_id[SLOW_LANE_NODES * SLOW_TPB];
    __shared__ uint8_t c_rc[SLOW_LANE_NODES * SLOW_TPB], c_strand[SLOW_LANE_NODES * SLOW_TPB];
    const uint32_t lane = threadIdx.x;
#ifdef SVJG_TIMING
    unsigned long long lstamp = __builtin_readcyclecounter();
#define ltick(i) do { const unsigned long long t_ = __builtin_readcyclecounter(); if ((a.diag & 16u) && lane == 0) atomicAdd(&a.dbg[24 + (i)], t_ - lstamp); lstamp = t_; } while (0)
#else
#define ltick(i) do { } while (0)
#endif
    for (uint64_t b0 = (uint64_t)blockIdx.x * SLOW_TPB; b0 < n_def; b0 += (uint64_t)gridDim.x * SLOW_TPB) {
        const bool have = b0 + lane < n_def;
        ltick(4);
        uint64_t s = 0, e = 0;
        if (have) {
            s = a.deferred[b0 + lane];
            e = ~0ull;
            for (uint64_t p = s & ~15ull; e == ~0ull; p += 16) {
                const uint4 v = *(const uint4 *)(a.gaf + p);
                uint32_t m = eq_mask16(v, 0x0A0A0A0Au) | eq_mask16(v, 0x0D0D0D0Du);
                if (p + 16 > a.n_bytes) m |= p >= a.n_bytes ? 0xFFFFu : (0xFFFFu << (a.n_bytes - p)) & 0xFFFFu;
                if (p < s) m &= 0xFFFFu << (s - p);
                if (m) e = p + (uint64_t)__builtin_ctz(m);
            }
        }
        const uint64_t a0 = s & ~15ull;
        const uint64_t span = have ? ((e - a0 + 15) & ~15ull) : 0;
        const uint32_t want = span <= (SLOW_MAXLINE < SLOW_LANE_LDS ? SLOW_MAXLINE : SLOW_LANE_LDS) ? (uint32_t)span : 0u;
        uint32_t tot;
        const uint32_t off = wave_excl_scan(want, tot);
        const bool staged = have && want && off + want <= SLOW_LANE_LDS;
        if (staged)
            for (uint32_t o = 0; o < want; o += 16) *(uint4 *)(stage + off + o) = *(const uint4 *)(a.gaf + a0 + o);
        __syncthreads();
        ltick(0);
        if (have) {
            SlowEmit em{&a, a.base_offset + s};
            int rc;
            if (staged) {
                typedef const __attribute__((address_space(3))) uint8_t *lds_text;
                const lds_text t = (lds_text)(stage + off);
                SlowLine ln;
                rc = slow_prologue(t, s - a0, s - a0 + (e - s), ln);
                ltick(1);
                if (!rc && ln.k >= 2) {
                    if (ln.k <= SLOW_LANE_NODES) {
                        NodeScratch ns{(SVJG_TAB_AS uint32_t *)c_id + lane, (SVJG_TAB_AS int64_t *)c_len + lane, (SVJG_TAB_AS uint8_t *)c_rc + lane, (SVJG_TAB_AS uint8_t *)c_strand + lane, SLOW_LANE_NODES, SLOW_TPB};
                        uint64_t order = 0;
                        rc = slow_wave_phase1(a.g, t, ln, ns, 0u, 1u, &order);
                        ltick(2);
                        if (!rc) rc = slow_wave_phase2(a.g, ln, ns, em, 0u, 1u, &order);
                        ltick(3);
                    } else rc = slow_line(a.g, t, s - a0, s - a0 + (e - s), em);
                }
            } else rc = slow_line(a.g, a.gaf, s, e, em);
            if (rc) report_line(a, a.base_offset + s, rc);
        }
        __syncthreads();
    }
}

constexpr uint32_t SLOW_NODES = 736;

__device__ inline uint32_t eq_bytes8(uint64_t w, uint32_t c) {
    const uint64_t x = w ^ (0x0101010101010101ull * c);
    const uint64_t z = ~((((x & 0x7F7F7F7F7F7F7F7Full) + 0x7F7F7F7F7F7F7F7Full) | x)) & 0x8080808080808080ull;
    return (uint32_t)(((z >> 7) * 0x0102040810204080ull) >> 56);
}
template <class Emit>
__device__ inline int slow_wave_links_summed(const GraphView &g, const SlowLine &ln, const SVJG_TAB_AS uint32_t *id, const SVJG_TAB_AS int64_t *P,
                                             const SVJG_TAB_AS uint8_t *strand, const SVJG_TAB_AS uint32_t *first, Emit &emit, uint32_t lane, uint64_t *order) {
    const uint64_t tot = (uint64_t)P[ln.k - 1];
    for (uint32_t i = lane; i + 1 < ln.k; i += 64) {
        const uint32_t lid = id[i], rid = id[i + 1];
        if (lid == NONE32 || rid == NONE32) continue;
        const uint32_t ei = edge_find(g, lid, strand[i], rid, strand[i + 1]);
        if (ei == NONE32) continue;
        const svjg_edge ed = g.edges[ei];
        const uint32_t nh = ed.meta >> 2;
        if (!nh) continue;
        if (g.dover_list) { *order = (2ull << 32) | i; return SVJG_EXC_TYPE_ERROR; }
        const uint32_t il = first[i], ir = first[i + 1];
        const int64_t left = P[il], right = (int64_t)(tot - (ir ? (uint64_t)P[ir - 1] : 0ull));
        if (left - ln.Ts >= (int64_t)g.d_over && right - (ln.Tlen - ln.Te - 1) >= (int64_t)g.d_over)
            for (uint32_t j = 0; j < nh; ++j) { uint32_t hv = edge_hit(g, ed, j); emit(hv >> 1, hv & 1u); }
    }
    return 0;
}

typedef const __attribute__((address_space(3))) uint8_t *slow_lds_text;
__device__ inline int slow_prologue_wave(slow_lds_text t, uint64_t s, uint64_t e, SlowLine &o, uint32_t lane) {
    o.k = 0;
    while (e > s && py_strip_space(t[e - 1])) --e;
    uint32_t tp[12], nt = 0;
#pragma unroll
    for (int i = 0; i < 12; ++i) tp[i] = (uint32_t)e;
    for (uint64_t base = s; base < e && nt < 12; base += 1024) {
        const uint64_t p = base + (uint64_t)lane * 16;
        uint32_t m = 0;
        if (p < e) {
            m = eq_bytes8(ld64(t, p), '\t') | (eq_bytes8(ld64(t, p + 8), '\t') << 8);
            if (p + 16 > e) m &= (1u << (e - p)) - 1u;
        }
        for (;;) {
            const unsigned long long hit = __ballot(m != 0);
            if (!hit || nt >= 12) break;
            const int L = __builtin_ctzll(hit);
            const uint32_t pos = (uint32_t)(base + (uint64_t)L * 16) + (uint32_t)__builtin_ctz((uint32_t)__shfl((int)m, L));
#pragma unroll
            for (int i = 0; i < 12; ++i) if ((uint32_t)i == nt) tp[i] = pos;
            ++nt;
            if ((int)lane == L) m &= m - 1u;
        }
    }
    if (nt < 11) return SVJG_EXC_VALUE_ERROR;
    auto fs = [&](int i) -> uint64_t { return i ? (uint64_t)tp[i - 1] + 1 : s; };
    auto fe = [&](int i) -> uint64_t { return (uint64_t)tp[i]; };
    int64_t v6 = 0, v7 = 0, v8 = 0, v10 = 0;
    {
        int64_t v = 0;
#define SVJG_COL(c, keep) do { const int r_ = py_int(t, fs(c), fe(c), v); if (r_ != PY_INT_OK) return r_ == PY_INT_BIG || has_high(t, fs(c), fe(c)) ? SVJG_EXC_ASK_HOST : SVJG_EXC_VALUE_ERROR; keep; } while (0)
        SVJG_COL(1, (void)0); SVJG_COL(2, (void)0); SVJG_COL(3, (void)0); SVJG_COL(6, v6 = v); SVJG_COL(7, v7 = v); SVJG_COL(8, v8 = v);
        SVJG_COL(9, (void)0); SVJG_COL(10, v10 = v); SVJG_COL(11, (void)0);
#undef SVJG_COL
    }
    {
        unsigned long long mine = 0;
        for (uint64_t base = s; base + 5 <= e; base += 1024) {
            const uint64_t p = base + (uint64_t)lane * 16;
            if (p + 5 <= e) {
                uint32_t m = eq_bytes8(ld64(t, p), 'i') | (eq_bytes8(ld64(t, p + 8), 'i') << 8);
                if (p + 16 + 4 > e) m &= (1u << (e - 4 - p)) - 1u;
                for (; m; m &= m - 1u) {
                    const uint64_t q = p + (uint32_t)__builtin_ctz(m);
                    if (t[q + 1] == 'd' && t[q + 2] == ':' && t[q + 3] == 'f' && t[q + 4] == ':') mine = q + 1;
                }
            }
        }
#pragma unroll
        for (int d = 32; d; d >>= 1) { const unsigned long long y = __shfl_xor(mine, d); mine = y > mine ? y : mine; }
        if (mine) {
            uint64_t a = mine - 1 + 5, b = a;
            while (b < e && t[b] != '\t') ++b;
            if (!py_float_ok(t, a, b)) return has_high(t, a, b) ? SVJG_EXC_ASK_HOST : SVJG_EXC_VALUE_ERROR;
        } else if (v10 == 0) return SVJG_EXC_ZERO_DIVISION;
    }
    o.ps = fs(5); o.pe = fe(5);
    if (o.pe == o.ps) return SVJG_EXC_INDEX_ERROR;
    o.oriented = t[o.ps] == '<' || t[o.ps] == '>';
    o.Tlen = v6; o.Ts = v7; o.Te = v8;
    return 0;
}
__global__ __launch_bounds__(SLOW_TPB) void k_classify_slow_wave(ClassifyArgs a, uint64_t n_def_arg, uint64_t lo, uint64_t hi) {
    const uint64_t n_def = slow_n_def(a, n_def_arg, lo, hi);
    __shared__ __attribute__((aligned(16))) uint8_t stage[SLOW_LDS];
    __shared__ int64_t n_len[SLOW_NODES];
    __shared__ uint32_t n_id[SLOW_NODES];
    __shared__ uint8_t n_rc[SLOW_NODES], n_strand[SLOW_NODES];
    __shared__ uint32_t n_piece[SLOW_NODES];
    __shared__ uint16_t n_colon[SLOW_NODES];
    __shared__ uint64_t n_key[SLOW_NODES];
    const uint32_t lane = threadIdx.x;
#ifdef SVJG_TIMING
    unsigned long long wstamp = __builtin_readcyclecounter();
#define wtick(i) do { const unsigned long long t_ = __builtin_readcyclecounter(); if ((a.diag & 16u) && lane == 0) atomicMax(&a.dbg[16 + (i)], t_ - wstamp); wstamp = t_; } while (0)
#else
#define wtick(i) do { } while (0)
#endif
    for (uint64_t b = blockIdx.x; b < n_def; b += gridDim.x) {
        const uint64_t s = a.deferred[b];
        wtick(7);
        const uint64_t a0 = s & ~15ull;
        uint64_t e = ~0ull;
        for (uint64_t p0 = a0; e == ~0ull; p0 += 1024) {
            const uint64_t p = p0 + lane * 16;
            const uint4 v = *(const uint4 *)(a.gaf + (p < a.n_bytes + 16 ? p : a0));
            uint32_t m = eq_mask16(v, 0x0A0A0A0Au) | eq_mask16(v, 0x0D0D0D0Du);
            if (p + 16 > a.n_bytes) m |= p >= a.n_bytes ? 0xFFFFu : (0xFFFFu << (a.n_bytes - p)) & 0xFFFFu;
            if (p < s) m &= 0xFFFFu << (s - p);
            const unsigned long long hit = __ballot(m != 0);
            if (hit) {
                const int first = __builtin_ctzll(hit);
                e = p0 + (uint64_t)first * 16 + (uint64_t)__builtin_ctz((uint32_t)__shfl((int)m, first));
            }
        }
        const uint64_t span = (e - a0 + 15) & ~15ull;
        const bool staged = span <= SLOW_LDS;
        if (staged) for (uint64_t o = (uint64_t)lane * 16; o < span; o += 1024) *(uint4 *)(stage + o) = *(const uint4 *)(a.gaf + a0 + o);
        __syncthreads();
        wtick(0);
        SlowEmit em{&a, a.base_offset + s};
        uint64_t order = 0;
        int rc = 0;
        auto wave_min = [&](int r, uint64_t ord) {
            unsigned long long key = r ? ((ord << 3) | (unsigned long long)r) : ~0ull;
#pragma unroll
            for (int d = 32; d; d >>= 1) { const unsigned long long y = __shfl_xor(key, d); key = y < key ? y : key; }
            return key == ~0ull ? 0 : (int)(key & 7ull);
        };
        if (staged) {
            typedef const __attribute__((address_space(3))) uint8_t *lds_text;
            const lds_text t = (lds_text)stage;
            SlowLine ln;
            rc = slow_prologue_wave(t, s - a0, s - a0 + (e - s), ln, lane);
            wtick(1);
            if (!rc) {
                const uint8_t sep1 = ln.oriented ? '<' : ',', sep2 = ln.oriented ? '>' : ',';
                uint32_t run = 0;
                for (uint64_t base = ln.ps; base < ln.pe; base += 64) {
                    const uint64_t q = base + lane;
                    bool st = false;
                    if (q < ln.pe) {
                        const uint8_t c = t[q], pc = q > ln.ps ? (uint8_t)t[q - 1] : sep1;
                        st = c != sep1 && c != sep2 && (pc == sep1 || pc == sep2);
                    }
                    const unsigned long long m = __ballot(st);
                    if (st) { const uint32_t i = run + (uint32_t)__popcll(m & ((1ull << lane) - 1ull)); if (i < SLOW_NODES) n_piece[i] = (uint32_t)q; }
                    run += (uint32_t)__popcll(m);
                }
                ln.k = run;
                __syncthreads();
            }
            if (!rc && ln.k >= 2) {
                if (ln.k <= SLOW_NODES) {
                    NodeScratch ns{(SVJG_TAB_AS uint32_t *)n_id, (SVJG_TAB_AS int64_t *)n_len, (SVJG_TAB_AS uint8_t *)n_rc, (SVJG_TAB_AS uint8_t *)n_strand, SLOW_NODES};
                    {
                        const uint8_t sep1 = ln.oriented ? '<' : ',', sep2 = ln.oriented ? '>' : ',';
                        for (uint32_t i = lane; i < ln.k; i += 64) {
                            const uint32_t s0 = n_piece[i];
                            uint32_t e0 = i + 1 < ln.k ? n_piece[i + 1] - 1u : (uint32_t)ln.pe;
                            while (e0 > s0 && ((uint8_t)t[e0 - 1] == sep1 || (uint8_t)t[e0 - 1] == sep2)) --e0;
                            n_len[i] = (int64_t)(e0 - s0);
                        }
                        __syncthreads();
                        for (uint32_t i = lane; i < ln.k; i += 64) { const uint16_t cw = piece_colons(t, n_piece[i], (uint64_t)n_len[i]); n_colon[i] = cw; n_key[i] = piece_key(t, n_piece[i], cw); n_piece[i] |= (uint32_t)n_len[i] << 16; }
                        __syncthreads();
                    }
                    wtick(2);
                    slow_wave_resolve(a.g, t, ln, ns, lane, 64u, (const SVJG_TAB_AS uint32_t *)n_piece);
                    __syncthreads();
                    bool clean = ln.oriented, rises = true;
                    for (uint32_t i = lane; i < ln.k; i += 64) {
                        const uint32_t x = n_id[i];
                        clean = clean && slow_node_clean(a.g, x);
                        rises = rises && x != NONE32 && (i == 0 || (n_id[1] > n_id[0] ? x > n_id[i - 1] : x < n_id[i - 1]));
                    }
                    clean = __ballot(!clean) == 0ull;
                    rises = __ballot(!rises) == 0ull;
                    const int r1 = slow_wave_strands(t, ln, ns, lane, 64u, &order, (const SVJG_TAB_AS uint32_t *)n_piece, (const SVJG_TAB_AS uint16_t *)n_colon, (const SVJG_TAB_AS uint64_t *)n_key, clean, rises);
                    rc = wave_min(r1, order);
                    __syncthreads();
                    wtick(3);
                    if (!rc) {
                        bool good = true, oneway = true;
                        for (uint32_t i = lane; i < ln.k; i += 64) {
                            const uint32_t x = n_id[i];
                            good = good && n_rc[i] == 0;
                            oneway = oneway && x != NONE32 && (i == 0 || (n_id[1] > n_id[0] ? x > n_id[i - 1] : x < n_id[i - 1]));
                        }
                        if (__ballot(!good) == 0ull) {
                            oneway = __ballot(!oneway) == 0ull;
                            __syncthreads();
                            for (uint32_t j = lane; j < ln.k; j += 64) {
                                uint32_t f = j;
                                if (!oneway) { const uint32_t x = n_id[j]; if (x != NONE32) { f = 0; while (n_id[f] != x) ++f; } }
                                n_piece[j] = f;
                            }
                            const uint32_t per = (ln.k + 63u) / 64u, j0 = lane * per < ln.k ? lane * per : ln.k, j1 = j0 + per < ln.k ? j0 + per : ln.k;
                            unsigned long long sum = 0;
                            for (uint32_t j = j0; j < j1; ++j) sum += (unsigned long long)n_len[j];
                            unsigned long long inc = sum;
#pragma unroll
                            for (int d = 1; d < 64; d <<= 1) { const unsigned long long y = __shfl_up(inc, d); if ((int)lane >= d) inc += y; }
                            unsigned long long run = inc - sum;
                            for (uint32_t j = j0; j < j1; ++j) { run += (unsigned long long)n_len[j]; n_len[j] = (int64_t)run; }
                            __syncthreads();
                            const int r2 = slow_wave_links_summed(a.g, ln, (const SVJG_TAB_AS uint32_t *)n_id, (const SVJG_TAB_AS int64_t *)n_len, (const SVJG_TAB_AS uint8_t *)n_strand,
                                                                  (const SVJG_TAB_AS uint32_t *)n_piece, em, lane, &order);
                            rc = wave_min(r2, order);
                        } else { const int r2 = slow_wave_phase2(a.g, ln, ns, em, lane, 64u, &order); rc = wave_min(r2, order); }
                    }
                    wtick(4);
                } else { const int r3 = slow_line(a.g, t, s - a0, s - a0 + (e - s), em, lane, 64u, &order); rc = wave_min(r3, order); }
            }
        } else { const int r4 = slow_line(a.g, a.gaf, s, e, em, lane, 64u, &order); rc = wave_min(r4, order); }
        if (lane == 0 && rc) report_line(a, a.base_offset + s, rc);
        __syncthreads();
    }
}

__global__ __launch_bounds__(TPB) void k_counts_guard(unsigned long long *counts, uint32_t n_slots, const DevStatus *st) {
    uint32_t mr = 0, ma = 0;
    for (uint32_t i = blockIdx.x * TPB + threadIdx.x; i < n_slots; i += gridDim.x * TPB) {
        const unsigned long long c = counts[i];
        const uint32_t r = (uint32_t)c, al = (uint32_t)(c >> 32);
        mr = r > mr ? r : mr; ma = al > ma ? al : ma;
    }
    for (int d = 32; d; d >>= 1) { const uint32_t y = __shfl_down(mr, d), z = __shfl_down(ma, d); mr = mr > y ? mr : y; ma = ma > z ? ma : z; }
    if ((threadIdx.x & 63) == 0) {
        if (mr) atomicMax(&counts[n_slots + GUARD_MAX_REF], (unsigned long long)mr);
        if (ma) atomicMax(&counts[n_slots + GUARD_MAX_ALT], (unsigned long long)ma);
    }
    if (st && blockIdx.x == 0 && threadIdx.x == 0) counts[n_slots + GUARD_REPEAT] = pass_repeat_word(st->overflow);
}


constexpr uint32_t LF_BLOCK = 1024;

__global__ __launch_bounds__(LF_BLOCK) void k_logfact_local(dd *tab, dd *bsum, uint32_t n) {
    __shared__ dd sh[LF_BLOCK];
    uint32_t i = blockIdx.x * LF_BLOCK + threadIdx.x;
    double v = (i >= 2 && i < n) ? log10((double)i) : 0.0;
    sh[threadIdx.x] = dd{v, 0.0};
    __syncthreads();
    for (uint32_t d = 1; d < LF_BLOCK; d <<= 1) {
        dd x = sh[threadIdx.x], y = dd{0.0, 0.0};
        if (threadIdx.x >= d) y = sh[threadIdx.x - d];
        __syncthreads();
        sh[threadIdx.x] = dd_add(x, y);
        __syncthreads();
    }
    if (i < n) tab[i] = sh[threadIdx.x];
    if (threadIdx.x == LF_BLOCK - 1) bsum[blockIdx.x] = sh[threadIdx.x];
}

__global__ void k_logfact_bsum(dd *bsum, uint32_t nb) {
    if (threadIdx.x || blockIdx.x) return;
    dd run{0.0, 0.0};
    for (uint32_t b = 0; b < nb; ++b) { dd t = bsum[b]; bsum[b] = run; run = dd_add(run, t); }
}

__global__ __launch_bounds__(LF_BLOCK) void k_logfact_add(dd *tab, const dd *bsum, uint32_t n) {
    uint32_t i = blockIdx.x * LF_BLOCK + threadIdx.x;
    if (i < n && blockIdx.x) tab[i] = dd_add(tab[i], bsum[blockIdx.x]);
}

struct GenoArgs {
    const unsigned long long *counts;
    const uint8_t *sv_type; const uint32_t *slot; const uint8_t *ok;
    uint64_t n_rows; uint32_t min_support;
    double l_ok, l_err, l_half;
    const dd *logfact; uint32_t logfact_n;
    uint8_t *gt; int64_t *pl; uint32_t *raw; uint8_t *genotyped;
    uint8_t *boundary;
    int32_t *pl32;
    unsigned int *max_n;
    uint32_t n_slots;
};

__device__ inline bool geno_gate(const GenoArgs &a, uint64_t r, uint32_t &ref, uint32_t &alt) {
    ref = alt = 0;
    const uint32_t ok = a.ok[r], sl = a.slot[r];
    if (sl != NONE32 && sl >= a.n_slots) { atomicOr(a.max_n + 1, 1u); return false; }
    if (!(ok & 1u) || sl == NONE32) return false;
    unsigned long long c = a.counts[sl];
    ref = (uint32_t)c; alt = (uint32_t)(c >> 32);
    return (ok & 2u) || (ref | alt) != 0;
}

__global__ __launch_bounds__(TPB) void k_geno_maxn(GenoArgs a) {
    uint64_t r = (uint64_t)blockIdx.x * TPB + threadIdx.x;
    uint32_t n = 0;
    if (r < a.n_rows) {
        uint32_t ref, alt;
        if (geno_gate(a, r, ref, alt)) {
            double c1, c2; uint32_t r1, r2; geno_counts(a.sv_type[r], ref, alt, c1, c2, r1, r2);
            const uint64_t n64 = geno_n(r1, r2);
            if (r1 && r2 && n64 < LOGFACT_CAP) n = (uint32_t)n64;
        }
    }
    for (int d = 32; d; d >>= 1) { uint32_t y = __shfl_down(n, d); n = n > y ? n : y; }
    if ((threadIdx.x & 63) == 0 && n) atomicMax(a.max_n, n);
}

__global__ __launch_bounds__(TPB) void k_genotype(GenoArgs a) {
  for (uint64_t r = (uint64_t)blockIdx.x * blockDim.x + threadIdx.x; r < a.n_rows; r += (uint64_t)gridDim.x * blockDim.x) {
    uint32_t ref, alt;
    bool go = geno_gate(a, r, ref, alt);
    a.raw[r * 2] = go ? ref : 0; a.raw[r * 2 + 1] = go ? alt : 0;
    a.genotyped[r] = go;
    a.boundary[r] = 0;
    if (!go) { a.gt[r] = 3; a.pl[r * 3] = a.pl[r * 3 + 1] = a.pl[r * 3 + 2] = 0; if (a.pl32) a.pl32[r * 3] = a.pl32[r * 3 + 1] = a.pl32[r * 3 + 2] = 0; continue; }
    GenoRow o;
    const uint32_t st = geno_row(a.sv_type[r], ref, alt, a.min_support, a.l_ok, a.l_err, a.l_half, a.logfact, a.logfact_n, o);
    if (st == GENO_ROW_GROW) atomicMax(a.max_n, (uint32_t)o.n);
    a.gt[r] = o.gt;
    bool wide = false;
#pragma unroll
    for (int i = 0; i < 3; ++i) {
        const int64_t v = o.pl[i];
        a.pl[r * 3 + i] = v;
        if (a.pl32) { a.pl32[r * 3 + i] = (int32_t)v; if (v != (int64_t)(int32_t)v) wide = true; }
    }
    if (wide) a.genotyped[r] = 3;
    if (o.near) a.boundary[r] = 1;
  }
}

}
```

### svjedi-graph_amd/svjg/capi.py

```python
import ctypes
import os
import sys

import numpy as np

HERE = os.path.dirname(os.path.abspath(__file__))
LIB_PATH = os.path.join(os.path.dirname(HERE), "csrc", "libsvjg_hip.so")
HOST_LIB_PATH = os.path.join(os.path.dirname(HERE), "csrc", "libsvjg_host.so")

HITREC_DT = np.dtype([("line_start", "<u8"), ("slot", "<u4"), ("n_ref", "<u2"), ("n_alt", "<u2")])

EXC_CLASS = {1: ValueError, 2: IndexError, 3: KeyError, 4: ZeroDivisionError, 6: TypeError}
LINE_ERRORS = (ValueError, IndexError, KeyError, ZeroDivisionError, TypeError)
DOVER_TYPE_ERROR = "'>=' not supported between instances of 'int' and 'list'"


class SvjgError(RuntimeError):
    pass


class CGraph(ctypes.Structure):
    _fields_ = [
        ("nodes", ctypes.c_void_p), ("n_nodes", ctypes.c_uint64),
        ("edges", ctypes.c_void_p), ("n_edges", ctypes.c_uint64),
        ("hits", ctypes.c_void_p), ("n_hits", ctypes.c_uint64),
        ("chrom_names", ctypes.c_char_p), ("chrom_off", ctypes.c_void_p), ("chrom_node_lo", ctypes.c_void_p),
        ("n_chrom", ctypes.c_uint32),
        ("n_slots", ctypes.c_uint32), ("d_over", ctypes.c_uint32), ("flags", ctypes.c_uint32),
    ]


class CStats(ctypes.Structure):
    _fields_ = [("n_lines", ctypes.c_uint64), ("n_deferred", ctypes.c_uint64), ("n_hitrecs", ctypes.c_uint64),
                ("non_ascii", ctypes.c_uint64)]


def cgraph_of(g):
    return CGraph(
        g.nodes.ctypes.data, g.n_nodes, g.edges.ctypes.data, g.n_edges, g.hits.ctypes.data, g.n_hits,
        g.chrom_names, g.chrom_off.ctypes.data, g.chrom_lo.ctypes.data, len(g.chroms),
        g.n_slots, g.d_over, g.flags)


_SIGS = {
    "svjg_abi_version": (ctypes.c_int, []),
    "svjg_device_count": (ctypes.c_int, []),
    "svjg_init": (ctypes.c_int, [ctypes.c_int, ctypes.POINTER(ctypes.c_void_p)]),
    "svjg_destroy": (None, [ctypes.c_void_p]),
    "svjg_last_error": (ctypes.c_char_p, [ctypes.c_void_p]),
    "svjg_load_graph": (ctypes.c_int, [ctypes.c_void_p, ctypes.POINTER(CGraph)]),
    "svjg_release_host_tables": (None, []),
    "svjg_gaf_upload": (ctypes.c_int, [ctypes.c_void_p, ctypes.c_void_p, ctypes.c_uint64]),
    "svjg_gaf_upload_part": (ctypes.c_int, [ctypes.c_void_p, ctypes.c_void_p, ctypes.c_uint64, ctypes.c_uint64, ctypes.c_uint64, ctypes.c_int]),
    "svjg_comm_set_stream": (ctypes.c_int, [ctypes.c_void_p, ctypes.c_int]),
    "svjg_copy_rate": (ctypes.c_int, [ctypes.c_void_p, ctypes.c_uint64, ctypes.POINTER(ctypes.c_double), ctypes.POINTER(ctypes.c_double)]),
    "svjg_classify_resident": (ctypes.c_int, [ctypes.c_void_p, ctypes.c_uint64, ctypes.c_int]),
    "svjg_classify": (ctypes.c_int, [ctypes.c_void_p, ctypes.c_void_p, ctypes.c_uint64, ctypes.c_uint64, ctypes.c_int]),
    "svjg_gaf_upload_file": (ctypes.c_int, [ctypes.c_void_p, ctypes.c_char_p, ctypes.c_uint64, ctypes.c_uint64]),
    "svjg_classify_file": (ctypes.c_int, [ctypes.c_void_p, ctypes.c_char_p, ctypes.c_uint64, ctypes.c_uint64, ctypes.c_int]),
    "svjg_reset_counts": (ctypes.c_int, [ctypes.c_void_p]),
    "svjg_get_stats": (ctypes.c_int, [ctypes.c_void_p, ctypes.POINTER(CStats)]),
    "svjg_get_defer_causes": (ctypes.c_int, [ctypes.c_void_p, ctypes.c_void_p]),
    "svjg_input_error": (ctypes.c_int, [ctypes.c_void_p, ctypes.POINTER(ctypes.c_int), ctypes.POINTER(ctypes.c_uint64)]),
    "svjg_get_counts": (ctypes.c_int, [ctypes.c_void_p, ctypes.c_void_p, ctypes.c_uint32]),
    "svjg_set_counts": (ctypes.c_int, [ctypes.c_void_p, ctypes.c_void_p, ctypes.c_uint32]),
    "svjg_alloc_counts": (ctypes.c_int, [ctypes.c_void_p, ctypes.c_uint32]),
    "svjg_get_hits": (ctypes.c_int, [ctypes.c_void_p, ctypes.c_void_p, ctypes.c_uint64, ctypes.POINTER(ctypes.c_uint64)]),
    "svjg_get_host_lines": (ctypes.c_int, [ctypes.c_void_p, ctypes.c_void_p, ctypes.c_uint64, ctypes.POINTER(ctypes.c_uint64)]),
    "svjg_comm_unique_id": (ctypes.c_int, [ctypes.c_char_p]),
    "svjg_comm_init": (ctypes.c_int, [ctypes.c_void_p, ctypes.c_char_p, ctypes.c_int, ctypes.c_int]),
    "svjg_allreduce_counts": (ctypes.c_int, [ctypes.c_void_p]),
    "svjg_comm_init_all": (ctypes.c_int, [ctypes.POINTER(ctypes.c_void_p), ctypes.c_int]),
    "svjg_comm_error": (ctypes.c_int, [ctypes.c_char_p, ctypes.c_uint64]),
    "svjg_allreduce_counts_all": (ctypes.c_int, [ctypes.POINTER(ctypes.c_void_p), ctypes.c_int]),
    "svjg_genotype": (ctypes.c_int, [ctypes.c_void_p, ctypes.c_void_p, ctypes.c_void_p, ctypes.c_void_p, ctypes.c_uint64,
                                     ctypes.c_uint32, ctypes.c_double, ctypes.c_void_p, ctypes.c_void_p, ctypes.c_void_p,
                                     ctypes.c_void_p]),
    "svjg_genotype_view": (ctypes.c_int, [ctypes.c_void_p, ctypes.c_void_p, ctypes.c_void_p, ctypes.c_void_p, ctypes.c_uint64,
                                          ctypes.c_uint32, ctypes.c_double] + [ctypes.POINTER(ctypes.c_void_p)] * 4),
    "svjg_set_rows": (ctypes.c_int, [ctypes.c_void_p, ctypes.c_void_p, ctypes.c_void_p, ctypes.c_void_p, ctypes.c_uint64]),
    "svjg_run_resident": (ctypes.c_int, [ctypes.c_void_p, ctypes.c_uint64, ctypes.c_uint32, ctypes.c_double] + [ctypes.POINTER(ctypes.c_void_p)] * 5),
    "svjg_run_begin": (ctypes.c_int, [ctypes.c_void_p, ctypes.c_uint64, ctypes.c_uint32, ctypes.c_double]),
    "svjg_run_end": (ctypes.c_int, [ctypes.c_void_p] + [ctypes.POINTER(ctypes.c_void_p)] * 5),
    "svjg_genotype_boundary": (ctypes.c_int, [ctypes.c_void_p, ctypes.c_void_p, ctypes.c_uint64]),
    "svjg_last_kernel_ms": (ctypes.c_int, [ctypes.c_void_p, ctypes.POINTER(ctypes.c_float), ctypes.POINTER(ctypes.c_float),
                                           ctypes.POINTER(ctypes.c_float)]),
    "svjg_sync": (ctypes.c_int, [ctypes.c_void_p]),
}

EXPORTS = tuple(_SIGS) + ("svjg_write_informative_json", "svjg_count_informative_json", "svjg_host_free",
                          "svjg_graph_load", "svjg_graph_view", "svjg_graph_info", "svjg_graph_free",
                          "svjg_vcf_load", "svjg_vcf_arrays", "svjg_vcf_write", "svjg_vcf_free")
_lib = None
_host_lib = None


def load_host_library():
    global _host_lib
    if _host_lib is None:
        if not os.path.exists(HOST_LIB_PATH):
            raise SvjgError(f"{HOST_LIB_PATH} not found: build it first (python __graft_entry__.py build)")
        lib = ctypes.CDLL(HOST_LIB_PATH)
        lib.svjg_write_informative_json.restype = ctypes.c_int
        lib.svjg_write_informative_json.argtypes = [ctypes.c_char_p, ctypes.c_void_p, ctypes.c_uint64, ctypes.c_void_p, ctypes.c_uint64,
                                                    ctypes.POINTER(ctypes.c_char_p), ctypes.c_uint32, ctypes.c_int]
        lib.svjg_count_informative_json.restype = ctypes.c_int
        lib.svjg_count_informative_json.argtypes = [ctypes.c_char_p, ctypes.POINTER(ctypes.c_void_p), ctypes.POINTER(ctypes.c_uint64),
                                                    ctypes.POINTER(ctypes.c_void_p), ctypes.POINTER(ctypes.c_uint64)]
        lib.svjg_host_free.restype = None
        lib.svjg_host_free.argtypes = [ctypes.c_void_p]
        lib.svjg_graph_load.restype = ctypes.c_int
        lib.svjg_graph_load.argtypes = [ctypes.c_char_p, ctypes.c_char_p, ctypes.POINTER(ctypes.c_void_p)]
        lib.svjg_graph_view.restype = ctypes.POINTER(CGraph)
        lib.svjg_graph_view.argtypes = [ctypes.c_void_p]
        lib.svjg_graph_info.restype = ctypes.c_int
        lib.svjg_graph_info.argtypes = [ctypes.c_void_p, ctypes.POINTER(ctypes.c_void_p), ctypes.POINTER(ctypes.c_uint64), ctypes.POINTER(ctypes.c_uint32)]
        lib.svjg_graph_free.restype = None
        lib.svjg_graph_free.argtypes = [ctypes.c_void_p]
        lib.svjg_vcf_load.restype = ctypes.c_int
        lib.svjg_vcf_load.argtypes = [ctypes.c_char_p, ctypes.c_char_p, ctypes.c_uint64, ctypes.c_void_p, ctypes.c_uint32, ctypes.c_int,
                                      ctypes.POINTER(ctypes.c_void_p)]
        lib.svjg_vcf_arrays.restype = ctypes.c_int
        lib.svjg_vcf_arrays.argtypes = [ctypes.c_void_p] + [ctypes.POINTER(ctypes.c_void_p)] * 3 + [ctypes.POINTER(ctypes.c_uint64)]
        lib.svjg_vcf_write.restype = ctypes.c_int
        lib.svjg_vcf_write.argtypes = [ctypes.c_void_p, ctypes.c_char_p] + [ctypes.c_void_p] * 4 + [ctypes.POINTER(ctypes.c_uint64)]
        lib.svjg_vcf_free.restype = None
        lib.svjg_vcf_free.argtypes = [ctypes.c_void_p]
        _host_lib = lib
    return _host_lib


class NativeVcfRows:

    def __init__(self, lib, h):
        self.lib, self.h = lib, h
        p = [ctypes.c_void_p() for _ in range(3)]
        n = ctypes.c_uint64(0)
        lib.svjg_vcf_arrays(h, ctypes.byref(p[0]), ctypes.byref(p[1]), ctypes.byref(p[2]), ctypes.byref(n))
        n = n.value

        def arr(ptr, dt):
            return np.frombuffer(ctypes.string_at(ptr, n * np.dtype(dt).itemsize), dtype=dt).copy() if n else np.zeros(0, dtype=dt)
        self.sv_type, self.slot, self.ok = arr(p[0], np.uint8), arr(p[1], np.uint32), arr(p[2], np.uint8)

    def write(self, out_path, gt, pl, raw, done):
        gt = np.ascontiguousarray(gt, dtype=np.uint8); pl = np.ascontiguousarray(pl, dtype=np.int64)
        raw = np.ascontiguousarray(raw, dtype=np.uint32); done = np.ascontiguousarray(done, dtype=np.uint8)
        n = len(self.sv_type)
        if len(gt) != n or pl.shape != (n, 3) or raw.shape != (n, 2) or len(done) != n:
            raise ValueError("result arrays do not match the rows")
        nd = ctypes.c_uint64(0)
        rc = self.lib.svjg_vcf_write(self.h, os.fsencode(out_path), gt.ctypes.data, pl.ctypes.data, raw.ctypes.data, done.ctypes.data, ctypes.byref(nd))
        if rc:
            raise OSError(f"cannot write {out_path} ({rc})")
        return nd.value

    def close(self):
        if self.h:
            self.lib.svjg_vcf_free(self.h)
            self.h = None

    def __del__(self):
        try:
            self.close()
        except Exception:
            pass


def vcf_load_native(vcf_path, keys, slots=None, slot_is_presence=False):
    lib = load_host_library()
    keys = list(keys)
    try:
        blob = ("\0".join(keys) + "\0").encode("ascii") if keys else b""
    except UnicodeEncodeError:
        return None
    if blob.count(b"\0") != len(keys):
        return None
    sl = None if slots is None else np.ascontiguousarray(slots, dtype=np.uint32)
    h = ctypes.c_void_p()
    rc = lib.svjg_vcf_load(os.fsencode(vcf_path), blob, len(blob), None if sl is None else sl.ctypes.data, len(keys), int(slot_is_presence), ctypes.byref(h))
    if rc == -11:
        return None
    if rc:
        raise SvjgError(f"svjg_vcf_load failed ({rc})")
    return NativeVcfRows(lib, h)


def graph_load_native(edges_json, gfa):
    lib = load_host_library()
    h = ctypes.c_void_p()
    rc = lib.svjg_graph_load(os.fsencode(edges_json), os.fsencode(gfa), ctypes.byref(h))
    if rc == -11:
        return None
    if rc:
        raise OSError(f"cannot read {edges_json} / {gfa}")
    try:
        v = lib.svjg_graph_view(h).contents
        from .graph import NODE_DT, EDGE_DT

        def arr(ptr, n, dt):
            if n == 0:
                return np.zeros(0, dtype=dt)
            return np.frombuffer(ctypes.string_at(ptr, n * np.dtype(dt).itemsize), dtype=dt).copy()
        n_chrom = v.n_chrom
        names_ptr = ctypes.c_void_p.from_buffer(v, type(v).chrom_names.offset).value
        chrom_off = arr(v.chrom_off, n_chrom + 1, np.uint32)
        blob, blen, nhz = ctypes.c_void_p(), ctypes.c_uint64(0), ctypes.c_uint32(0)
        lib.svjg_graph_info(h, ctypes.byref(blob), ctypes.byref(blen), ctypes.byref(nhz))
        sv = ctypes.string_at(blob, blen.value).decode("ascii").split("\0")[:-1] if blen.value else []
        return dict(
            nodes=arr(v.nodes, v.n_nodes + 1, NODE_DT), n_nodes=int(v.n_nodes),
            edges=arr(v.edges, max(1, v.n_edges), EDGE_DT), n_edges=int(v.n_edges),
            hits=arr(v.hits, max(1, v.n_hits), np.uint32), n_hits=int(v.n_hits),
            chrom_names=ctypes.string_at(names_ptr, int(chrom_off[-1]) + 4), chrom_off=chrom_off,
            chrom_lo=arr(v.chrom_node_lo, n_chrom + 1, np.uint32), sv_ids=sv, n_hazard=int(nhz.value))
    finally:
        lib.svjg_graph_free(h)


def count_informative_json(path):
    lib = load_host_library()
    kp, cp = ctypes.c_void_p(), ctypes.c_void_p()
    kl, nk = ctypes.c_uint64(0), ctypes.c_uint64(0)
    rc = lib.svjg_count_informative_json(os.fsencode(path), ctypes.byref(kp), ctypes.byref(kl), ctypes.byref(cp), ctypes.byref(nk))
    if rc == -10:
        raise ValueError(f"{path}: not the JSON written by filter-alignments.py")
    if rc:
        raise OSError(f"cannot read {path}")
    try:
        blob = ctypes.string_at(kp, kl.value)
        keys = [k.decode("utf-8") for k in blob.split(b"\0")[:-1]] if kl.value else []
        if nk.value:
            cnt = np.ctypeslib.as_array(ctypes.cast(cp, ctypes.POINTER(ctypes.c_uint64)), shape=(nk.value * 2,)).copy()
        else:
            cnt = np.zeros(0, dtype=np.uint64)
    finally:
        lib.svjg_host_free(kp); lib.svjg_host_free(cp)
    if (cnt >= 2 ** 32).any():
        raise ValueError("list too long")
# ... 84 lines not shown
        self._chk(self.lib.svjg_alloc_counts(self.h, n_slots))

    def upload(self, gaf):
        a = _as_u8(gaf)
        self._chk(self.lib.svjg_gaf_upload(self.h, a.ctypes.data if a.size else None, a.size))

    def upload_parts(self, parts, capacity_bytes):
        at, prev = 0, None
        for p in parts:
            if prev is not None:
                self._chk(self.lib.svjg_gaf_upload_part(self.h, prev.ctypes.data if prev.size else None, prev.size, at, capacity_bytes, 0))
                at += int(prev.size)
            prev = _as_u8(p)
        if prev is None:
            prev = np.zeros(0, dtype=np.uint8)
        self._chk(self.lib.svjg_gaf_upload_part(self.h, prev.ctypes.data if prev.size else None, prev.size, at, capacity_bytes, 1))
        return at + int(prev.size)

    def allreduce_on_second_stream(self, on):
        self._chk(self.lib.svjg_comm_set_stream(self.h, 1 if on else 0))

    def copy_rate(self, n_bytes=1 << 31):
        v, r = ctypes.c_double(0), ctypes.c_double(0)
        self._chk(self.lib.svjg_copy_rate(self.h, n_bytes, ctypes.byref(v), ctypes.byref(r)))
        return v.value, r.value

    def classify_resident(self, base_offset=0, want_hits=False):
        self._chk(self.lib.svjg_classify_resident(self.h, base_offset, int(want_hits)))

    def classify(self, gaf, base_offset=0, want_hits=False):
        a = _as_u8(gaf)
        self._chk(self.lib.svjg_classify(self.h, a.ctypes.data if a.size else None, a.size, base_offset, int(want_hits)))

    def classify_file(self, path, offset, n_bytes, want_hits=False):
        rc = self.lib.svjg_classify_file(self.h, os.fsencode(path), offset, n_bytes, int(want_hits))
        if rc == -6:
            raise OSError(self.lib.svjg_last_error(self.h).decode())
        self._chk(rc)

    def reset_counts(self):
        self._chk(self.lib.svjg_reset_counts(self.h))

    def stats(self):
        s = CStats()
        self._chk(self.lib.svjg_get_stats(self.h, ctypes.byref(s)))
        return {"n_lines": s.n_lines, "n_deferred": s.n_deferred, "n_hitrecs": s.n_hitrecs, "non_ascii": s.non_ascii}

    def defer_causes(self):
        out = np.zeros(8, dtype=np.uint64)
        self._chk(self.lib.svjg_get_defer_causes(self.h, out.ctypes.data))
        return dict(zip(("columns", "id_tag_filter", "long_path", "node_name", "whole_stripe"), (int(x) for x in out[:5])))

    def counts(self):
        out = np.zeros((self.n_slots, 2), dtype=np.uint32)
        self._chk(self.lib.svjg_get_counts(self.h, out.ctypes.data, self.n_slots))
        return out

    def set_counts(self, c):
        c = np.ascontiguousarray(c, dtype=np.uint32)
        assert c.shape == (self.n_slots, 2)
        self._chk(self.lib.svjg_set_counts(self.h, c.ctypes.data, self.n_slots))

    def hits(self, out=None):
        n = self.stats()["n_hitrecs"]
        if out is None:
            out = np.empty(n, dtype=HITREC_DT)
        assert out.dtype == HITREC_DT and out.flags["C_CONTIGUOUS"] and len(out) == n
        got = ctypes.c_uint64(0)
        self._chk(self.lib.svjg_get_hits(self.h, out.ctypes.data, n, ctypes.byref(got)))
        assert got.value == n
        return out

    def host_lines(self):
        n = ctypes.c_uint64(0)
        self._chk(self.lib.svjg_get_host_lines(self.h, None, 0, ctypes.byref(n)))
        out = np.zeros(n.value, dtype=np.uint64)
        if n.value:
            self._chk(self.lib.svjg_get_host_lines(self.h, out.ctypes.data, n.value, ctypes.byref(n)))
        return np.sort(out)

    def comm_init(self, unique_id, n_ranks, rank):
        self._chk(self.lib.svjg_comm_init(self.h, unique_id, n_ranks, rank))

    def allreduce_counts(self):
        self._chk(self.lib.svjg_allreduce_counts(self.h))

    def genotype(self, sv_type, slot, ok, min_support, err, reuse_outputs=False):
        n = len(sv_type)
        sv_type = np.ascontiguousarray(sv_type, dtype=np.uint8)
        slot = np.ascontiguousarray(slot, dtype=np.uint32)
        ok = np.ascontiguousarray(ok, dtype=np.uint8)
        if reuse_outputs and n:
            p = [ctypes.c_void_p() for _ in range(4)]
            self._chk(self.lib.svjg_genotype_view(self.h, sv_type.ctypes.data, slot.ctypes.data, ok.ctypes.data, n, min_support,
                                                  float(err), *[ctypes.byref(x) for x in p]))

            def view(ptr, count, dt):
                a = np.frombuffer((ctypes.c_char * (count * np.dtype(dt).itemsize)).from_address(ptr.value), dtype=dt)
                a.flags.writeable = False
                return a
            return view(p[0], n, np.uint8), view(p[1], n * 3, np.int64).reshape(n, 3), view(p[2], n * 2, np.uint32).reshape(n, 2), view(p[3], n, np.uint8)
        gt = np.empty(n, dtype=np.uint8)
        pl = np.empty((n, 3), dtype=np.int64)
        raw = np.empty((n, 2), dtype=np.uint32)
        done = np.empty(n, dtype=np.uint8)
        self._chk(self.lib.svjg_genotype(self.h, sv_type.ctypes.data, slot.ctypes.data, ok.ctypes.data, n, min_support,
                                         float(err), gt.ctypes.data, pl.ctypes.data, raw.ctypes.data, done.ctypes.data))
        return gt, pl, raw, done

    def set_rows(self, sv_type, slot, ok):
        sv_type = np.ascontiguousarray(sv_type, dtype=np.uint8)
        slot = np.ascontiguousarray(slot, dtype=np.uint32)
        ok = np.ascontiguousarray(ok, dtype=np.uint8)
        self._n_rows = len(sv_type)
        self._chk(self.lib.svjg_set_rows(self.h, sv_type.ctypes.data, slot.ctypes.data, ok.ctypes.data, self._n_rows))

    def _run_views(self, p):
        n = self._n_rows
        if not n:
            self.last_boundary = np.zeros(0, np.uint8)
            return np.zeros(0, np.uint8), np.zeros((0, 3), np.int32), np.zeros((0, 2), np.uint32), np.zeros(0, np.uint8)

        def view(ptr, count, dt):
            a = np.frombuffer((ctypes.c_char * (count * np.dtype(dt).itemsize)).from_address(ptr.value), dtype=dt)
            a.flags.writeable = False
            return a
        self.last_boundary = view(p[4], n, np.uint8)
        return view(p[0], n, np.uint8), view(p[1], n * 3, np.int32).reshape(n, 3), view(p[2], n * 2, np.uint32).reshape(n, 2), view(p[3], n, np.uint8)

    def run_resident(self, min_support, err, base_offset=0):
        p = [ctypes.c_void_p() for _ in range(5)]
        self._chk(self.lib.svjg_run_resident(self.h, base_offset, min_support, float(err), *[ctypes.byref(x) for x in p]))
        return self._run_views(p)

    def run_begin(self, min_support, err, base_offset=0):
        self._chk(self.lib.svjg_run_begin(self.h, base_offset, min_support, float(err)))

    def run_end(self):
        p = [ctypes.c_void_p() for _ in range(5)]
        self._chk(self.lib.svjg_run_end(self.h, *[ctypes.byref(x) for x in p]))
        return self._run_views(p)

    def boundary_flags(self, n_rows):
        out = np.zeros(n_rows, dtype=np.uint8)
        if n_rows:
            self._chk(self.lib.svjg_genotype_boundary(self.h, out.ctypes.data, n_rows))
        return out

    def kernel_ms(self):
        a, b, c = ctypes.c_float(0), ctypes.c_float(0), ctypes.c_float(0)
        self._chk(self.lib.svjg_last_kernel_ms(self.h, ctypes.byref(a), ctypes.byref(b), ctypes.byref(c)))
        return a.value, b.value, c.value

    def sync(self):
        self._chk(self.lib.svjg_sync(self.h))


def release_host_tables():
    load_library().svjg_release_host_tables()


def device_count():
    return int(load_library().svjg_device_count())


def _handles(ctxs):
    return (ctypes.c_void_p * len(ctxs))(*[c.h for c in ctxs])


def comm_init_all(ctxs):
    rc = ctxs[0].lib.svjg_comm_init_all(_handles(ctxs), len(ctxs))
    if rc:
        buf = ctypes.create_string_buffer(512)
        ctxs[0].lib.svjg_comm_error(buf, 512)
        raise SvjgError(f"libsvjg_hip error {rc}: {buf.value.decode(errors='replace')}")


def allreduce_counts_all(ctxs):
    ctxs[0]._chk(ctxs[0].lib.svjg_allreduce_counts_all(_handles(ctxs), len(ctxs)))


def unique_id():
    lib = load_library()
    buf = ctypes.create_string_buffer(128)
    rc = lib.svjg_comm_unique_id(buf)
    if rc:
        raise SvjgError(f"svjg_comm_unique_id failed ({rc})")
    return buf.raw


def _as_u8(x):
    if isinstance(x, np.ndarray):
        return np.ascontiguousarray(x.view(np.uint8))
    return np.frombuffer(x, dtype=np.uint8)
```

Baseline: 8.007 billion.

## Merge slow-path kernels into one exact kernel and prezero next pass counts

Replaces the two slow-path launches (wave and lane variants) with a single k_classify_exact kernel. It picks the wave or lane role on the device from the deferred count and runs two lane waves per block. The same kernel zeroes the counts and status of the next run slot, so the next pass can skip its reset kernel, and the run ring grows from two to three slots. Kernel timing now uses device wall-clock stamps by default instead of stream events, which removes event records from the stream. The cost is more LDS per block, a three-blocks-per-CU constraint, and more complex slot bookkeeping.

```diff
diff --git a/include/svjg.h b/include/svjg.h
--- a/include/svjg.h
+++ b/include/svjg.h
@@ -141,6 +141,7 @@
 void svjg_vcf_free(svjg_vcf *v);
 
 int svjg_last_kernel_ms(svjg_ctx *ctx, float *classify_main_ms, float *classify_slow_ms, float *genotype_ms);
+int svjg_last_main_ms(svjg_ctx *ctx, float *by_stamps, float *by_events);
 int svjg_sync(svjg_ctx *ctx);
 int svjg_copy_rate(svjg_ctx *ctx, uint64_t n_bytes, double *copy_gb_per_s, double *read_gb_per_s);
 
diff --git a/svjedi-graph_amd/csrc/svjg_capi.hip b/svjedi-graph_amd/csrc/svjg_capi.hip
--- a/svjedi-graph_amd/csrc/svjg_capi.hip
+++ b/svjedi-graph_amd/csrc/svjg_capi.hip
@@ -66,8 +66,11 @@
 constexpr int STAGE_THREADS = 4;
 constexpr uint64_t STAGE_PIECE = 8ull << 20;
 
+constexpr int RUN_SLOTS = 3;
+
 struct svjg_ctx {
     int device = 0;
+    int wall_khz = 0;
     int n_cu = 256;
     int occ_main = 0;
     hipStream_t stream = nullptr, copy_stream = nullptr;
@@ -101,12 +104,14 @@
         void *d = nullptr;  uint64_t d_cap = 0;  void *h = nullptr;  uint64_t h_cap = 0;  void *h_dev = nullptr;
         unsigned long long *counts = nullptr;  uint64_t counts_cap = 0;
         hipEvent_t ev[6] = {};  hipEvent_t computed = nullptr, copied = nullptr;
-        uint64_t base_offset = 0;  uint32_t min_support = 0;  double err = 0;  bool had_text = false, slow_end_own = false;
-    } run[2];
+        uint64_t base_offset = 0;  uint32_t min_support = 0;  double err = 0;  bool had_text = false, slow_end_own = false, timed_by_events = false;
+        bool clean = false;
+    } run[RUN_SLOTS];
     int run_head = 0, run_tail = 0, run_inflight = 0;
     int counts_in_slot = -1;
     void *d_run_in = nullptr;  uint64_t d_run_in_cap = 0;  uint64_t run_rows = 0;  bool have_rows = false;
     float ms_main = 0, ms_slow = 0, ms_geno = 0;
+    float ms_main_stamps = 0, ms_main_events = 0;
     ncclComm_t comm = nullptr;
     bool allreduce_second = false;
     uint64_t part_total = 0, part_need = 0, part_next = 0;
@@ -150,6 +155,7 @@
     }
     hipDeviceProp_t prop;
     if (hipGetDeviceProperties(&prop, device) == hipSuccess) c->n_cu = prop.multiProcessorCount;
+    if (hipDeviceGetAttribute(&c->wall_khz, hipDeviceAttributeWallClockRate, device) != hipSuccess || c->wall_khz < 1) c->wall_khz = 0;
     for (auto &ev : c->ev) hipEventCreate(&ev);
     if (hipMalloc(&c->d_dbg, 32 * 8) != hipSuccess || hipMalloc(&c->d_st, sizeof(DevStatus)) != hipSuccess || hipMalloc(&c->d_maxn, sizeof(unsigned int)) != hipSuccess ||
         hipHostMalloc((void **)&c->h_stp, 2 * sizeof(DevStatus), hipHostMallocDefault) != hipSuccess) {
@@ -171,6 +177,7 @@
     c->d_nodes = nullptr; c->d_edges = nullptr; c->d_hits = nullptr; c->d_cnames = nullptr; c->d_coff = nullptr;
     c->d_clo = nullptr; c->d_chash = nullptr; c->d_counts = nullptr; c->d_snap = nullptr;
     c->have_graph = false; c->have_counts = false;
+    for (auto &r : c->run) r.clean = false;
 }
 
 extern "C" void svjg_destroy(svjg_ctx *c) {
@@ -341,17 +348,6 @@
     for (int t = 0; t < STAGE_THREADS; ++t)
         if (rcs[t]) { c->err = errs[t]; return rcs[t]; }
     return 0;
-}
-
-static uint32_t lane_blocks_per_cu(svjg_ctx *c) {
-    static int per_cu = 0;
-    if (!per_cu) {
-        int n = 0;
-        if (hipOccupancyMaxActiveBlocksPerMultiprocessor(&n, k_classify_slow, (int)SLOW_TPB, 0) != hipSuccess || n < 1) n = 4;
-        per_cu = n;
-    }
-    (void)c;
-    return (uint32_t)per_cu;
 }
 
 static int gaf_finish(svjg_ctx *c, uint64_t n, uint64_t need) {
@@ -941,6 +937,11 @@
     return L;
 }
 
+static bool kernel_ms_by_events(const svjg_ctx *c) {
+    static const bool env_events = [] { const char *e = getenv("SVJG_KERNEL_MS"); return e && !strcmp(e, "events"); }();
+    return env_events || c->wall_khz == 0;
+}
+
 extern "C" int svjg_set_rows(svjg_ctx *c, const uint8_t *sv_type, const uint32_t *slot, const uint8_t *ok, uint64_t n_rows) {
     if (!c || (n_rows && (!sv_type || !slot || !ok))) return SVJG_E_ARG;
     if (c->run_inflight) { c->err = "svjg_set_rows with a pass in flight"; return SVJG_E_ARG; }
@@ -950,8 +951,9 @@
     const RunLayout L = run_layout(n_rows);
     int rc;
     if ((rc = ensure(c, &c->d_run_in, &c->d_run_in_cap, n_rows * 6 + 64, 1, false))) return rc;
-    for (int k = 0; k < 2; ++k) {
+    for (int k = 0; k < RUN_SLOTS; ++k) {
         svjg_ctx::RunSlot &r = c->run[k];
+        r.clean = false;
         if ((rc = ensure(c, &r.d, &r.d_cap, L.total, 1, false))) return rc;
         if (L.out_bytes > r.h_cap) {
             if (r.h) hipHostFree(r.h);
@@ -1012,12 +1014,14 @@
     DevStatus *d_st = (DevStatus *)(base + L.status);
     if (r.counts_cap < (uint64_t)c->n_slots + GUARD_WORDS) { c->err = "svjg_set_rows must follow svjg_load_graph"; return SVJG_E_ARG; }
     GenoArgs ga = run_geno_args(c, r, L, min_support, err, r.counts);
-    {
-        const uint64_t words = (uint64_t)c->n_slots + GUARD_WORDS;
+    const uint64_t words = (uint64_t)c->n_slots + GUARD_WORDS;
+    if (!r.clean) {
         uint32_t rg = (uint32_t)((words + TPB - 1) / TPB);
         if (rg > 1024) rg = 1024;
         hipLaunchKernelGGL(k_step_reset, dim3(rg), dim3(TPB), 0, c->stream, r.counts, words, d_st, ga.max_n);
     }
+    r.clean = false;
+    r.timed_by_events = kernel_ms_by_events(c);
     const uint64_t max_blocks = (uint64_t)c->n_cu * 4, wave_limit = 16 * max_blocks;
     if (n) {
         ClassifyArgs a{};
@@ -1026,13 +1030,17 @@
         main_launch_setup(c, 0, n, base_offset, 0, a, grid, lds);
         if (!a.long_pre) { c->err = "no memory for the workers' scratch words"; return SVJG_E_NOMEM; }
         a.st = d_st; a.counts = r.counts;
-        HIPCHK(c, hipEventRecord(r.ev[0], c->stream));
+        if (r.timed_by_events) HIPCHK(c, hipEventRecord(r.ev[0], c->stream));
         hipLaunchKernelGGL(k_classify_main, dim3(grid), dim3(WG), lds, c->stream, a);
-        HIPCHK(c, hipEventRecord(r.ev[1], c->stream));
-        hipLaunchKernelGGL(k_classify_slow_wave, dim3((uint32_t)c->n_cu), dim3(SLOW_TPB), 0, c->stream, a, SLOW_ASK_DEVICE, 0ull, wave_limit);
-        const uint64_t lane_blocks = (uint64_t)c->n_cu * lane_blocks_per_cu(c);
-        hipLaunchKernelGGL(k_classify_slow, dim3((uint32_t)lane_blocks), dim3(SLOW_TPB), 0, c->stream, a, SLOW_ASK_DEVICE, wave_limit, ~0ull - 1);
+        if (r.timed_by_events) HIPCHK(c, hipEventRecord(r.ev[1], c->stream));
+        svjg_ctx::RunSlot &nxt = c->run[(c->run_head + 1) % RUN_SLOTS];
+        NextPass nx{};
+        if (nxt.d && nxt.counts && nxt.counts_cap >= words) {
+            nx.counts = nxt.counts; nx.n_words = words; nx.st = (DevStatus *)((uint8_t *)nxt.d + L.status); nx.max_n = (unsigned int *)((uint8_t *)nxt.d + L.maxn);
+        }
+        hipLaunchKernelGGL(k_classify_exact, dim3((uint32_t)c->n_cu * EXACT_BLOCKS_PER_CU), dim3(EXACT_TPB), 0, c->stream, a, wave_limit, nx);
         HIPCHK(c, hipGetLastError());
+        nxt.clean = nx.counts != nullptr;
     }
     static const bool env_second = [] { const char *e = getenv("SVJG_ALLREDUCE_STREAM"); return e && !strcmp(e, "second"); }();
     const bool allreduce_second = env_second || c->allreduce_second;
@@ -1046,7 +1054,7 @@
     };
     r.slow_end_own = false;
     if (c->comm && !allreduce_second) {
-        if (r.had_text) { HIPCHK(c, hipEventRecord(r.ev[2], c->stream)); r.slow_end_own = true; }
+        if (n && r.timed_by_events) { HIPCHK(c, hipEventRecord(r.ev[2], c->stream)); r.slow_end_own = true; }
         if ((rc = reduce_on(c->stream))) return rc;
     }
     HIPCHK(c, hipEventRecord(r.computed, c->stream));
@@ -1067,7 +1075,7 @@
     HIPCHK(c, hipEventRecord(r.copied, c->copy_stream));
     c->counts_in_slot = c->run_head;
     r.had_text = n != 0;
-    c->run_head ^= 1; ++c->run_inflight;
+    c->run_head = (c->run_head + 1) % RUN_SLOTS; ++c->run_inflight;
     return 0;
 }
 
@@ -1077,7 +1085,7 @@
     if (!c->run_inflight) { c->err = "no pass in flight"; return SVJG_E_ARG; }
     HIPCHK(c, hipSetDevice(c->device));
     svjg_ctx::RunSlot &r = c->run[c->run_tail];
-    c->run_tail ^= 1; --c->run_inflight;
+    c->run_tail = (c->run_tail + 1) % RUN_SLOTS; --c->run_inflight;
     const uint64_t n = c->gaf_bytes, n_rows = c->run_rows;
     const RunLayout L = run_layout(n_rows);
     uint8_t *hb = (uint8_t *)r.h;
@@ -1087,8 +1095,17 @@
     c->hs() = *(const DevStatus *)(tail + L.status);
     c->ms_slow = 0;
     if (r.had_text) {
-        HIPCHK(c, hipEventElapsedTime(&c->ms_main, r.ev[0], r.ev[1]));
-        if (c->hs().n_deferred) HIPCHK(c, hipEventElapsedTime(&c->ms_slow, r.ev[1], r.slow_end_own ? r.ev[2] : r.computed));
+        const DevStatus &t = c->hs();
+        const float per_tick = c->wall_khz ? 1.0f / (float)c->wall_khz : 0.0f;
+        c->ms_main_stamps = t.t_last > t.t_first ? (float)(t.t_last - t.t_first) * per_tick : 0.0f;
+        c->ms_main_events = 0;
+        c->ms_main = c->ms_main_stamps;
+        if (t.n_deferred && t.t_exact > t.t_last) c->ms_slow = (float)(t.t_exact - t.t_last) * per_tick;
+        if (r.timed_by_events) {
+            HIPCHK(c, hipEventElapsedTime(&c->ms_main_events, r.ev[0], r.ev[1]));
+            c->ms_main = c->ms_main_events;
+            if (t.n_deferred) HIPCHK(c, hipEventElapsedTime(&c->ms_slow, r.ev[1], r.slow_end_own ? r.ev[2] : r.computed));
+        }
     }
     if (n_rows) HIPCHK(c, hipEventElapsedTime(&c->ms_geno, r.ev[4], r.ev[5]));
     bool again = false;
@@ -1151,6 +1168,13 @@
     if (m) *m = c->ms_main;
     if (s) *s = c->ms_slow;
     if (g) *g = c->ms_geno;
+    return 0;
+}
+
+extern "C" int svjg_last_main_ms(svjg_ctx *c, float *by_stamps, float *by_events) {
+    if (!c) return SVJG_E_ARG;
+    if (by_stamps) *by_stamps = c->ms_main_stamps;
+    if (by_events) *by_events = c->ms_main_events;
     return 0;
 }
 
diff --git a/svjedi-graph_amd/csrc/svjg_kernels.h b/svjedi-graph_amd/csrc/svjg_kernels.h
--- a/svjedi-graph_amd/csrc/svjg_kernels.h
+++ b/svjedi-graph_amd/csrc/svjg_kernels.h
@@ -70,6 +70,8 @@
     unsigned long long next_chunk;
     unsigned long long n_host;
     unsigned long long cause[8];
+    unsigned long long t_first, t_last;
+    unsigned long long t_exact;
 };
 
 struct ClassifyArgs {
@@ -346,6 +348,7 @@
 __device__ inline unsigned long long low_bits64(uint32_t n) { return n >= 64u ? ~0ull : ((1ull << n) - 1ull); }
 __device__ inline uint32_t clamp64(uint32_t hi, uint32_t lo) { return hi > lo ? (hi - lo < 64u ? hi - lo : 64u) : 0u; }
 
+static_assert(KLONG <= 224, "ids + bitmap share the 256 tab-bitmap words");
 __device__ inline bool long_line_may_repeat(uint32_t *ids, uint32_t K, uint32_t lane) {
     const uint32_t nb = K <= 128u ? 128u : K <= 192u ? 64u : 32u, B = nb * 32u;
     uint32_t *bm = ids + 256u - nb;
@@ -391,6 +394,7 @@
     const GraphView g = a.g;
 
     unsigned long long pos = a.begin + (unsigned long long)blockIdx.x * a.region;
+    if (blockIdx.x == 0 && lane == 0) a.st->t_first = wall_clock64();
     if (pos >= a.n_bytes) return;
     unsigned long long rend = pos + a.region < a.n_bytes ? pos + a.region : a.n_bytes;
 
@@ -1157,6 +1161,7 @@
     rend = pos + a.small < a.n_bytes ? pos + a.small : a.n_bytes;
   }
     if (lane == 0 && wave_lines) atomicAdd(&a.st->n_lines, wave_lines);
+    if (lane == 0) atomicMax(&a.st->t_last, (unsigned long long)wall_clock64());
 #ifdef SVJG_TIMING
     if ((a.diag & 16u) && lane == 0)
         for (int i = 0; i < 16; ++i) atomicAdd(&a.dbg[i], acc[i]);
@@ -1232,20 +1237,24 @@
     return (n > lo && n <= hi) ? n : 0;
 }
 constexpr uint32_t SLOW_LANE_NODES = 12;
-__global__ __launch_bounds__(SLOW_TPB) void k_classify_slow(ClassifyArgs a, uint64_t n_def_arg, uint64_t lo, uint64_t hi) {
-    const uint64_t n_def = slow_n_def(a, n_def_arg, lo, hi);
-    __shared__ __attribute__((aligned(16))) uint8_t stage[SLOW_LANE_LDS];
-    __shared__ int64_t c_len[SLOW_LANE_NODES * SLOW_TPB];
-    __shared__ uint32_t c_id[SLOW_LANE_NODES * SLOW_TPB];
-    __shared__ uint8_t c_rc[SLOW_LANE_NODES * SLOW_TPB], c_strand[SLOW_LANE_NODES * SLOW_TPB];
-    const uint32_t lane = threadIdx.x;
+constexpr uint32_t SLOW_LANE_SCRATCH = SLOW_LANE_NODES * SLOW_TPB * 14;
+template <uint32_t WAVES, uint32_t STAGE>
+__device__ __forceinline__ void slow_lane_role(const ClassifyArgs &a, const uint64_t n_def, uint8_t *pool) {
+    static_assert(STAGE % 16 == 0, "LDS alignment");
+    const uint32_t lane = threadIdx.x & 63u, wave = WAVES > 1 ? threadIdx.x >> 6 : 0u;
+    uint8_t *stage = pool + wave * (STAGE + SLOW_LANE_SCRATCH);
+    int64_t *c_len = (int64_t *)(stage + STAGE);
+    uint32_t *c_id = (uint32_t *)(c_len + SLOW_LANE_NODES * SLOW_TPB);
+    uint8_t *c_rc = (uint8_t *)(c_id + SLOW_LANE_NODES * SLOW_TPB), *c_strand = c_rc + SLOW_LANE_NODES * SLOW_TPB;
+    constexpr uint32_t SLOW_LANE_LDS = STAGE;
 #ifdef SVJG_TIMING
     unsigned long long lstamp = __builtin_readcyclecounter();
 #define ltick(i) do { const unsigned long long t_ = __builtin_readcyclecounter(); if ((a.diag & 16u) && lane == 0) atomicAdd(&a.dbg[24 + (i)], t_ - lstamp); lstamp = t_; } while (0)
 #else
 #define ltick(i) do { } while (0)
 #endif
-    for (uint64_t b0 = (uint64_t)blockIdx.x * SLOW_TPB; b0 < n_def; b0 += (uint64_t)gridDim.x * SLOW_TPB) {
+    for (uint64_t g0 = (uint64_t)blockIdx.x * WAVES; g0 * SLOW_TPB < n_def; g0 += (uint64_t)gridDim.x * WAVES) {
+        const uint64_t b0 = (g0 + wave) * SLOW_TPB;
         const bool have = b0 + lane < n_def;
         ltick(4);
         uint64_t s = 0, e = 0;
@@ -1295,6 +1304,10 @@
         __syncthreads();
     }
 }
+__global__ __launch_bounds__(SLOW_TPB) void k_classify_slow(ClassifyArgs a, uint64_t n_def_arg, uint64_t lo, uint64_t hi) {
+    __shared__ __attribute__((aligned(16))) uint8_t pool[SLOW_LANE_LDS + SLOW_LANE_SCRATCH];
+    slow_lane_role<1, SLOW_LANE_LDS>(a, slow_n_def(a, n_def_arg, lo, hi), pool);
+}
 
 constexpr uint32_t SLOW_NODES = 736;
 
@@ -1387,16 +1400,18 @@
     o.Tlen = v6; o.Ts = v7; o.Te = v8;
     return 0;
 }
-__global__ __launch_bounds__(SLOW_TPB) void k_classify_slow_wave(ClassifyArgs a, uint64_t n_def_arg, uint64_t lo, uint64_t hi) {
-    const uint64_t n_def = slow_n_def(a, n_def_arg, lo, hi);
-    __shared__ __attribute__((aligned(16))) uint8_t stage[SLOW_LDS];
-    __shared__ int64_t n_len[SLOW_NODES];
-    __shared__ uint32_t n_id[SLOW_NODES];
-    __shared__ uint8_t n_rc[SLOW_NODES], n_strand[SLOW_NODES];
-    __shared__ uint32_t n_piece[SLOW_NODES];
-    __shared__ uint16_t n_colon[SLOW_NODES];
-    __shared__ uint64_t n_key[SLOW_NODES];
-    const uint32_t lane = threadIdx.x;
+constexpr uint32_t SLOW_WAVE_BYTES = SLOW_LDS + SLOW_NODES * 28;
+template <bool SOLO> __device__ __forceinline__ void slow_role_sync() { if (SOLO) wave_sync(); else __syncthreads(); }
+template <bool SOLO>
+__device__ __forceinline__ void slow_wave_role(const ClassifyArgs &a, const uint64_t n_def, uint8_t *pool) {
+    uint8_t *stage = pool;
+    int64_t *n_len = (int64_t *)(pool + SLOW_LDS);
+    uint64_t *n_key = (uint64_t *)(n_len + SLOW_NODES);
+    uint32_t *n_id = (uint32_t *)(n_key + SLOW_NODES);
+    uint32_t *n_piece = n_id + SLOW_NODES;
+    uint16_t *n_colon = (uint16_t *)(n_piece + SLOW_NODES);
+    uint8_t *n_rc = (uint8_t *)(n_colon + SLOW_NODES), *n_strand = n_rc + SLOW_NODES;
+    const uint32_t lane = threadIdx.x & 63u;
 #ifdef SVJG_TIMING
     unsigned long long wstamp = __builtin_readcyclecounter();
 #define wtick(i) do { const unsigned long long t_ = __builtin_readcyclecounter(); if ((a.diag & 16u) && lane == 0) atomicMax(&a.dbg[16 + (i)], t_ - wstamp); wstamp = t_; } while (0)
@@ -1423,7 +1438,7 @@
         const uint64_t span = (e - a0 + 15) & ~15ull;
         const bool staged = span <= SLOW_LDS;
         if (staged) for (uint64_t o = (uint64_t)lane * 16; o < span; o += 1024) *(uint4 *)(stage + o) = *(const uint4 *)(a.gaf + a0 + o);
-        __syncthreads();
+        slow_role_sync<SOLO>();
         wtick(0);
         SlowEmit em{&a, a.base_offset + s};
         uint64_t order = 0;
@@ -1455,7 +1470,7 @@
                     run += (uint32_t)__popcll(m);
                 }
                 ln.k = run;
-                __syncthreads();
+                slow_role_sync<SOLO>();
             }
             if (!rc && ln.k >= 2) {
                 if (ln.k <= SLOW_NODES) {
@@ -1468,13 +1483,13 @@
                             while (e0 > s0 && ((uint8_t)t[e0 - 1] == sep1 || (uint8_t)t[e0 - 1] == sep2)) --e0;
                             n_len[i] = (int64_t)(e0 - s0);
                         }
-                        __syncthreads();
+                        slow_role_sync<SOLO>();
                         for (uint32_t i = lane; i < ln.k; i += 64) { const uint16_t cw = piece_colons(t, n_piece[i], (uint64_t)n_len[i]); n_colon[i] = cw; n_key[i] = piece_key(t, n_piece[i], cw); n_piece[i] |= (uint32_t)n_len[i] << 16; }
-                        __syncthreads();
+                        slow_role_sync<SOLO>();
                     }
                     wtick(2);
                     slow_wave_resolve(a.g, t, ln, ns, lane, 64u, (const SVJG_TAB_AS uint32_t *)n_piece);
-                    __syncthreads();
+                    slow_role_sync<SOLO>();
                     bool clean = ln.oriented, rises = true;
                     for (uint32_t i = lane; i < ln.k; i += 64) {
                         const uint32_t x = n_id[i];
@@ -1485,7 +1500,7 @@
                     rises = __ballot(!rises) == 0ull;
                     const int r1 = slow_wave_strands(t, ln, ns, lane, 64u, &order, (const SVJG_TAB_AS uint32_t *)n_piece, (const SVJG_TAB_AS uint16_t *)n_colon, (const SVJG_TAB_AS uint64_t *)n_key, clean, rises);
                     rc = wave_min(r1, order);
-                    __syncthreads();
+                    slow_role_sync<SOLO>();
                     wtick(3);
                     if (!rc) {
                         bool good = true, oneway = true;
@@ -1496,7 +1511,7 @@
                         }
                         if (__ballot(!good) == 0ull) {
                             oneway = __ballot(!oneway) == 0ull;
-                            __syncthreads();
+                            slow_role_sync<SOLO>();
                             for (uint32_t j = lane; j < ln.k; j += 64) {
                                 uint32_t f = j;
                                 if (!oneway) { const uint32_t x = n_id[j]; if (x != NONE32) { f = 0; while (n_id[f] != x) ++f; } }
@@ -1510,7 +1525,7 @@
                             for (int d = 1; d < 64; d <<= 1) { const unsigned long long y = __shfl_up(inc, d); if ((int)lane >= d) inc += y; }
                             unsigned long long run = inc - sum;
                             for (uint32_t j = j0; j < j1; ++j) { run += (unsigned long long)n_len[j]; n_len[j] = (int64_t)run; }
-                            __syncthreads();
+                            slow_role_sync<SOLO>();
                             const int r2 = slow_wave_links_summed(a.g, ln, (const SVJG_TAB_AS uint32_t *)n_id, (const SVJG_TAB_AS int64_t *)n_len, (const SVJG_TAB_AS uint8_t *)n_strand,
                                                                   (const SVJG_TAB_AS uint32_t *)n_piece, em, lane, &order);
                             rc = wave_min(r2, order);
@@ -1521,8 +1536,38 @@
             }
         } else { const int r4 = slow_line(a.g, a.gaf, s, e, em, lane, 64u, &order); rc = wave_min(r4, order); }
         if (lane == 0 && rc) report_line(a, a.base_offset + s, rc);
-        __syncthreads();
-    }
+        slow_role_sync<SOLO>();
+    }
+}
+__global__ __launch_bounds__(SLOW_TPB) void k_classify_slow_wave(ClassifyArgs a, uint64_t n_def_arg, uint64_t lo, uint64_t hi) {
+    __shared__ __attribute__((aligned(16))) uint8_t pool[SLOW_WAVE_BYTES];
+    slow_wave_role<false>(a, slow_n_def(a, n_def_arg, lo, hi), pool);
+}
+
+constexpr uint32_t EXACT_TPB = 2 * SLOW_TPB;
+constexpr uint32_t EXACT_LANE_STAGE = 16128;
+constexpr uint32_t EXACT_LANE_BYTES = 2 * (EXACT_LANE_STAGE + SLOW_LANE_SCRATCH);
+constexpr uint32_t EXACT_LDS = SLOW_WAVE_BYTES > EXACT_LANE_BYTES ? SLOW_WAVE_BYTES : EXACT_LANE_BYTES;
+constexpr uint32_t EXACT_BLOCKS_PER_CU = 3;
+static_assert(EXACT_LDS <= (128 / EXACT_BLOCKS_PER_CU) * LDS_GRANULE, "three blocks of k_classify_exact per CU");
+struct NextPass { unsigned long long *counts; uint64_t n_words; DevStatus *st; unsigned int *max_n; };
+__global__ __launch_bounds__(EXACT_TPB) void k_classify_exact(ClassifyArgs a, uint64_t wave_limit, NextPass nx) {
+    __shared__ __attribute__((aligned(16))) uint8_t pool[EXACT_LDS];
+    if (nx.counts) {
+        for (uint64_t i = (uint64_t)blockIdx.x * EXACT_TPB + threadIdx.x; i < nx.n_words; i += (uint64_t)gridDim.x * EXACT_TPB) nx.counts[i] = 0ull;
+        if (blockIdx.x == 0 && threadIdx.x == 0) {
+            DevStatus z{}; z.err = ~0ull;
+            *nx.st = z;
+            nx.max_n[0] = 0u; nx.max_n[1] = 0u;
+        }
+    }
+    const uint64_t n_def = slow_n_def(a, SLOW_ASK_DEVICE, 0ull, ~0ull - 1);
+    if (!n_def) return;
+    if (n_def <= wave_limit) {
+        if (threadIdx.x >= SLOW_TPB) return;
+        slow_wave_role<true>(a, n_def, pool);
+    } else slow_lane_role<2, EXACT_LANE_STAGE>(a, n_def, pool);
+    if ((threadIdx.x & 63u) == 0) atomicMax(&a.st->t_exact, (unsigned long long)wall_clock64());
 }
 
 __global__ __launch_bounds__(TPB) void k_counts_guard(unsigned long long *counts, uint32_t n_slots, const DevStatus *st) {
diff --git a/svjedi-graph_amd/svjg/capi.py b/svjedi-graph_amd/svjg/capi.py
--- a/svjedi-graph_amd/svjg/capi.py
+++ b/svjedi-graph_amd/svjg/capi.py
@@ -85,6 +85,7 @@
     "svjg_genotype_boundary": (ctypes.c_int, [ctypes.c_void_p, ctypes.c_void_p, ctypes.c_uint64]),
     "svjg_last_kernel_ms": (ctypes.c_int, [ctypes.c_void_p, ctypes.POINTER(ctypes.c_float), ctypes.POINTER(ctypes.c_float),
                                            ctypes.POINTER(ctypes.c_float)]),
+    "svjg_last_main_ms": (ctypes.c_int, [ctypes.c_void_p, ctypes.POINTER(ctypes.c_float), ctypes.POINTER(ctypes.c_float)]),
     "svjg_sync": (ctypes.c_int, [ctypes.c_void_p]),
 }
 
@@ -475,6 +476,11 @@
         self._chk(self.lib.svjg_last_kernel_ms(self.h, ctypes.byref(a), ctypes.byref(b), ctypes.byref(c)))
         return a.value, b.value, c.value
 
+    def main_ms_both(self):
+        a, b = ctypes.c_float(0), ctypes.c_float(0)
+        self._chk(self.lib.svjg_last_main_ms(self.h, ctypes.byref(a), ctypes.byref(b)))
+        return a.value, b.value
+
     def sync(self):
         self._chk(self.lib.svjg_sync(self.h))
 
```

Result: faster. 8.105 billion, median of 6 (+1.2%).
